# Anttwo/SuGaR

Hardware: AMD Instinct MI355X
Metric: train_step_images_per_sec (higher is better)
Workload: dtype f32; 1 GPU; metric: 1000000 Gaussians @ 1920x1080, SH degree 3, 3DGS train step (raster fwd -> 0.8 L1 + 0.2 DSSIM -> bwd -> Adam, 59 floats/Gaussian), 8 orbit cameras cycled; parallelism=view-sharded dp1, single process, no collective

## Files before the change

### include/sugar_raster.h

```cpp
#ifndef SUGAR_RASTER_H_INCLUDED
#define SUGAR_RASTER_H_INCLUDED

#include <stddef.h>
#include <stdint.h>

#ifdef __cplusplus
extern "C" {
#endif

#define SGR_ABI_VERSION 4

#define SGR_E_INVALID (-1)
#define SGR_E_HIP (-2)
#define SGR_E_ALLOC (-3)

typedef char* (*sgr_alloc_fn)(void* user, size_t bytes);

int sgr_abi_version(void);
const char* sgr_last_error(void);

int64_t sgr_forward(sgr_alloc_fn geom_alloc, void* geom_user,
                    sgr_alloc_fn binning_alloc, void* binning_user,
                    sgr_alloc_fn img_alloc, void* img_user,
                    int P, int D, int M,
// ... 13 lines not shown
#define SGR_HDR_L1_OVERFLOW 6
#define SGR_HDR_LAYOUT_CAP 8
#define SGR_HDR_DEEP 9
#define SGR_HDR_REPAIR 7
typedef struct sgr_forward_info {
    int binning_mode;
    int sync_free;
    int speculation;
} sgr_forward_info;
typedef struct sgr_forward_opts {
    int64_t binning_capacity;
    int flags;
    uint32_t* header_host;
    void* header_event;
    const uint32_t* tile_need;
    uint32_t* tile_need_out;
    float hint_margin;
    uint32_t chunk_grid;
    sgr_forward_info* info;
    const uint32_t* tile_order;
    uint32_t* tile_order_out;
} sgr_forward_opts;
int64_t sgr_forward_ex(sgr_alloc_fn geom_alloc, void* geom_user,
                       sgr_alloc_fn binning_alloc, void* binning_user,
                       sgr_alloc_fn img_alloc, void* img_user,
                       int P, int D, int M,
                       const float* background, int width, int height,
                       const float* means3D, const float* shs, const float* colors_precomp,
                       const float* opacities, const float* scales, float scale_modifier,
                       const float* rotations, const float* cov3D_precomp,
                       const float* viewmatrix, const float* projmatrix, const float* cam_pos,
                       float tan_fovx, float tan_fovy, int prefiltered,
                       float* out_color, int* radii, int debug, void* stream, const sgr_forward_opts* opts);

#define SGR_FLAG_RAW_PARAMS 1
#define SGR_FLAG_SINGLE_LEVEL_BINNING 2
#define SGR_FLAG_DEFER_POST 4
#define SGR_FLAG_SPECULATIVE 8
#define SGR_FLAG_EXACT_ALPHA 16
#define SGR_FLAG_NO_DEEP 32
#define SGR_FLAG_REACH 64
void sgr_set_deep_min(int entries);
int sgr_get_deep_min(void);
void sgr_set_exact_alpha(int on);
int sgr_get_exact_alpha(void);
#define SGR_MODE_RAW_PARAMS 4
#define SGR_MODE_SH_DIR_ELSEWHERE 8

int sgr_backward(int P, int D, int M, int64_t R,
                 const float* background, int width, int height,
                 const float* means3D, const float* shs, const float* colors_precomp,
                 const float* scales, float scale_modifier, const float* rotations,
                 const float* cov3D_precomp, const float* viewmatrix, const float* projmatrix,
                 const float* cam_pos, float tan_fovx, float tan_fovy, const int* radii,
                 char* geom_buffer, char* binning_buffer, char* img_buffer,
                 const float* dL_dpix,
                 float* dL_dmean2D, float* dL_dconic, float* dL_dopacity, float* dL_dcolor,
                 float* dL_dmean3D, float* dL_dcov3D, float* dL_dsh, float* dL_dscale, float* dL_drot,
                 int debug, void* stream);

int sgr_backward_phase(int phase, int P, int D, int M, int64_t R,
                       const float* background, int width, int height,
                       const float* means3D, const float* shs, const float* colors_precomp,
                       const float* scales, float scale_modifier, const float* rotations,
                       const float* cov3D_precomp, const float* viewmatrix, const float* projmatrix,
                       const float* cam_pos, float tan_fovx, float tan_fovy, const int* radii,
                       char* geom_buffer, char* binning_buffer, char* img_buffer,
                       const float* dL_dpix,
                       float* dL_dmean2D, float* dL_dconic, float* dL_dopacity, float* dL_dcolor,
                       float* dL_dmean3D, float* dL_dcov3D, float* dL_dsh, float* dL_dscale, float* dL_drot,
                       int debug, void* stream);

typedef struct sgr_backward_opts {
    float* max_radii2D;
    float* grad_accum;
    float* denom;
    float* campos_row;
    int flags;
} sgr_backward_opts;
#define SGR_BWD_EXACT_ALPHA 2
#define SGR_BWD_TILE_ORDER_READY 1
#define SGR_BWD_DENSE 8
#define SGR_BWD_ACC_CLEAN 4
int sgr_backward_ex(int phase, int P, int D, int M, int64_t R,
                    const float* background, int width, int height,
                    const float* means3D, const float* shs, const float* colors_precomp,
                    const float* scales, float scale_modifier, const float* rotations,
                    const float* cov3D_precomp, const float* viewmatrix, const float* projmatrix,
                    const float* cam_pos, float tan_fovx, float tan_fovy, const int* radii,
                    char* geom_buffer, char* binning_buffer, char* img_buffer,
                    const float* dL_dpix,
                    float* dL_dmean2D, float* dL_dconic, float* dL_dopacity, float* dL_dcolor,
                    float* dL_dmean3D, float* dL_dcov3D, float* dL_dsh, float* dL_dscale, float* dL_drot,
                    int debug, void* stream, const sgr_backward_opts* opts);

int sgr_sh_grad_from_views(int P, int n_views, int D, int M, const float* means3D, const float* campos_all,
                           const float* dcolor_all, int64_t view_stride, float* dL_dsh, void* stream);

int sgr_sh_adam_from_views(int P, int n_views, int D, int M, const float* means3D, const float* campos_all,
                           const float* dcolor_all, int64_t view_stride, float* sh_params, float* exp_avg, float* exp_avg_sq,
                           float lr_dc,
                           float lr_rest, float beta1, float beta2, float eps, int step, float grad_scale, void* stream);

int sgr_sh_adam_from_views_ex(int P, int n_views, int D, int M, const float* means3D, const float* campos_all,
                              const float* dcolor_all, int64_t view_stride, float* sh_params, float* exp_avg, float* exp_avg_sq,
                              float lr_dc, float lr_rest, float beta1, float beta2, float eps, int step, float grad_scale,
                              float* dmean_extra, void* stream);

int sgr_sh_adam_zero_grad(int P, int M, float* sh_params, float* exp_avg, float* exp_avg_sq, const uint8_t* reach, float lr_dc,
                          float lr_rest, float beta1, float beta2, float eps, int step, float grad_scale,
                          const uint32_t* guard_header, uint32_t guard_capacity, void* stream);
int sgr_sh_adam_from_views_masked(int P, int n_views, int D, int M, const float* means3D, const float* campos_all,
                                  const float* dcolor_all, int64_t view_stride, float* sh_params, float* exp_avg, float* exp_avg_sq,
                                  float lr_dc, float lr_rest, float beta1, float beta2, float eps, int step, float grad_scale,
                                  uint8_t* reach, const uint32_t* guard_header, uint32_t guard_capacity, void* stream);
void sgr_set_adam_overlap(int on);
int sgr_get_adam_overlap(void);
size_t sgr_geom_reach_offset_bytes(int P);

int sgr_mark_visible(int P, const float* means3D, const float* viewmatrix, const float* projmatrix,
                     uint8_t* present, void* stream);

size_t sgr_geom_bytes(int P);
size_t sgr_img_bytes(int width, int height);
size_t sgr_binning_bytes(int64_t R, int width, int height);

size_t sgr_geom_rec_offset(int P);
size_t sgr_geom_acc_offset_bytes(int P);
size_t sgr_img_final_T_offset(int width, int height);
size_t sgr_img_n_contrib_offset(int width, int height);
size_t sgr_img_tile_start_offset(int width, int height);
size_t sgr_img_tile_maxc_offset(int width, int height);
size_t sgr_img_tile_walked_offset(int width, int height);
size_t sgr_img_header_offset(int width, int height);
size_t sgr_binning_point_list_offset(int64_t R);

#define SGR_N_STAGES 15
void sgr_profile_enable(int stage_mask);
int sgr_profile_read(double* ms_sum, int64_t* count, int n_stages);


int sgr_dist2(int P, const float* points, float* meanDists, void* stream);
int sgr_knn(int N, const float* query, int M, const float* ref, int K, float* dists, int64_t* idx, void* stream);
size_t sgr_knn_grid_scratch_bytes(int M);
int sgr_knn_grid(int N, const float* query, int M, const float* ref, int K, float* dists, int64_t* idx, char* scratch,
                 void* stream);
int sgr_dist2_grid(int P, const float* points, float* meanDists, char* scratch, void* stream);

size_t sgr_l1_ssim_scratch_bytes(int channels, int width, int height);
int sgr_l1_ssim_forward(int channels, int width, int height, const float* img, const float* gt, float lambda,
                        char* scratch, float* loss_out, void* stream);
int sgr_l1_ssim_backward(int channels, int width, int height, const float* img, const float* gt, float lambda,
                         const char* scratch, const float* grad_loss, float* grad_img, void* stream);
int sgr_l1_ssim_backward_ex(int channels, int width, int height, const float* img, const float* gt, float lambda,
                            const char* scratch, const float* grad_loss, float* grad_img, float* loss_out, void* stream);

int sgr_adam_step(long long n, float* params, const float* grads, float* exp_avg, float* exp_avg_sq, int n_seg,
                  const long long* seg_begin, const long long* seg_end, const float* seg_lr_a, const float* seg_lr_b,
                  const int* seg_period, const int* seg_split, float beta1, float beta2, float eps, int step,
                  float grad_scale, void* stream);
int sgr_adam_step_multi(int n_tensors, const long long* n, float* const* params, const float* const* grads, float* const* exp_avg,
                        float* const* exp_avg_sq, const float* lr, const float* beta1, const float* beta2, const float* eps,
                        const int* step, void* stream);
int sgr_adam_step_ex(long long n, float* params, const float* grads, float* exp_avg, float* exp_avg_sq, int n_seg,
                     const long long* seg_begin, const long long* seg_end, const float* seg_lr_a, const float* seg_lr_b,
                     const int* seg_period, const int* seg_split, float beta1, float beta2, float eps, int step,
                     float grad_scale, const float* extra, long long extra_n, void* stream);

typedef struct sgr_train_config {
    int P, D, M, width, height;
    float* flat; float* flat_grad; float* exp_avg; float* exp_avg_sq;
    long long off_xyz, off_opacity, off_scaling, off_rotation, off_features, n_small;
    float lr_xyz, lr_opacity, lr_scaling, lr_rotation, lr_features_dc, lr_features_rest;
    float beta1, beta2, eps, lambda_dssim;
    const float* background;
    char* geom; size_t geom_bytes;
    char* img; size_t img_bytes;
    char* binning; size_t binning_bytes;
    int64_t binning_capacity;
    char* loss_scratch;
    float* image;
    float* grad_image;
    float* loss_out;
    float* colors;
    int* radii;
    uint32_t* header_host;
    float* dL_dmean2D;
    float* max_radii2D; float* grad_accum; float* denom;
} sgr_train_config;
typedef struct sgr_train_view {
    const float* viewmatrix; const float* projmatrix; const float* campos;
    float tan_fovx, tan_fovy;
    const float* gt_image;
    const uint32_t* tile_need;
    uint32_t* tile_need_out;
    float hint_margin;
    uint32_t chunk_grid;
    const uint32_t* tile_order;
    uint32_t* tile_order_out;
    uint32_t flags;
} sgr_train_view;
#define SGR_VIEW_DEEP_LISTS 1
typedef struct sgr_train_exchange {
    int n_views;
    const float* all_colors;
    int64_t view_stride;
    const float* all_campos;
    float grad_scale;
    int step;
    int64_t g_begin, g_end;
    int64_t f_begin, f_end;
} sgr_train_exchange;
typedef struct sgr_trainer sgr_trainer;
sgr_trainer* sgr_trainer_create(const sgr_train_config* cfg);
void sgr_trainer_destroy(sgr_trainer* t);
int sgr_trainer_set_binning(sgr_trainer* t, char* binning, size_t bytes, int64_t capacity);
int sgr_trainer_step(sgr_trainer* t, const sgr_train_view* view, int phases, const sgr_train_exchange* ex, void* stream);
int sgr_trainer_set_exchange_chunks(sgr_trainer* t, int n);
int sgr_trainer_forward_valid(sgr_trainer* t, uint32_t* header_out);
const char* sgr_trainer_last_error(void);
int sgr_trainer_acc_dirty(sgr_trainer* t);
int sgr_rccl_unique_id(char* out128);
int sgr_trainer_comm_init(sgr_trainer* t, const char* id128, int world, int rank, float* recv, size_t recv_bytes);
int sgr_trainer_comm_destroy(sgr_trainer* t);
int sgr_trainer_comm_abort(sgr_trainer* t);
int sgr_trainer_step_exchange(sgr_trainer* t, const sgr_train_view* view, int step, void* stream);
double sgr_trainer_last_exchange_wait_ms(sgr_trainer* t);
size_t sgr_bin2_bytes(int P, int width, int height);

int sgr_scaled_rotation_forward(int P, const float* quaternions, const float* scaling, int inverse_scales, float* out,
                                void* stream);
int sgr_scaled_rotation_backward(int P, const float* quaternions, const float* scaling, int inverse_scales,
                                 const float* dL_dout, float* dL_dquaternions, float* dL_dscaling, void* stream);

int sgr_pack_gaussians(int P, const float* centers, const float* inv_scaled_rot, const float* strengths, float* packed,
                       void* stream);
int sgr_density_field_forward(int N, int K, const float* x, const int64_t* nbr_idx, const float* centers,
                              const float* inv_scaled_rot, const float* strengths, float density_factor,
                              float* neighbor_opacities, float* density, const float* packed, void* stream);
int sgr_density_field_backward(int N, int K, const float* x, const int64_t* nbr_idx, const float* centers,
                               const float* inv_scaled_rot, const float* strengths, float density_factor,
                               const float* dL_dopacities, const float* dL_ddensity, float* dL_dx, float* dL_dcenters,
                               float* dL_dinv_scaled_rot, float* dL_dstrengths, const float* packed, void* stream);
size_t sgr_density_field_backward_scratch_bytes(int N, int K, int P);
int sgr_density_field_backward_gather(int N, int K, int P, const float* x, const int64_t* nbr_idx, const float* centers,
                                      const float* inv_scaled_rot, const float* strengths, float density_factor,
                                      const float* dL_dopacities, const float* dL_ddensity, float* dL_dx, float* dL_dcenters,
                                      float* dL_dinv_scaled_rot, float* dL_dstrengths, char* scratch, const float* packed, void* stream);

size_t sgr_scatter_add_rows_scratch_bytes(long long N, int P);
int sgr_scatter_add_rows(long long N, const int64_t* idx, const float* src, int W, int P, float* out, char* scratch, void* stream);

int sgr_sample_transform_forward(long long N, int P, const int64_t* idx, const float* points, const float* quaternions,
                                 const float* scaling, const float* noise, float factor, float* out, void* stream);
size_t sgr_sample_transform_backward_scratch_bytes(long long N, int P);
int sgr_sample_transform_backward(long long N, int P, const int64_t* idx, const float* quaternions, const float* scaling,
                                  const float* noise, float factor, const float* dL_dout, float* dL_dpoints, float* dL_dquaternions,
                                  float* dL_dscaling, char* scratch, void* stream);
int sgr_smallest_axis_forward(int P, const float* quaternions, const float* scaling, float* axis, int64_t* axis_idx, void* stream);
int sgr_smallest_axis_backward(int P, const float* quaternions, const float* scaling, const float* dL_daxis, float* dL_dquaternions,
                               void* stream);
int sgr_depth_lookup_forward(long long M, const float* points_cam, const float* projection, const float* depth, long long stride_y,
                             long long stride_x, int height, int width, float* out, void* stream);
int sgr_depth_lookup_backward(long long M, const float* points_cam, const float* projection, const float* depth, long long stride_y,
                              long long stride_x, int height, int width, const float* dL_dout, float* dL_dpoints_cam, float* dL_ddepth,
                              void* stream);
int sgr_sdf_field_forward(int N, int K, int P, const float* x, const int64_t* nbr_idx, const float* centers, const float* inv_scaled_rot,
                          const float* strengths, const float* min_scaling, float density_factor, float density_threshold,
                          float opacity_min_clamp, float* neighbor_opacities, float* density, float* beta, float* sdf,
                          const float* packed, void* stream);
size_t sgr_sdf_field_backward_scratch_bytes(int N, int K, int P);
int sgr_sdf_field_backward(int N, int K, int P, const float* x, const int64_t* nbr_idx, const float* centers, const float* inv_scaled_rot,
                           const float* strengths, float density_factor, float density_threshold, float opacity_min_clamp,
                           const float* density, const float* beta, const float* dL_dopacities, const float* dL_ddensity,
                           const float* dL_dbeta, const float* dL_dsdf, float* dL_dx, float* dL_dcenters, float* dL_dinv_scaled_rot,
                           float* dL_dstrengths, float* dL_dmin_scaling, char* scratch, const float* packed, void* stream);

#define SGR_CL_SQUARED_EST 1
#define SGR_CL_SQUARED_SURFACE 2
#define SGR_CL_WITH_EST 4
#define SGR_CL_WITH_SURFACE 8
int sgr_surface_band(int P, const float* points, const float* quaternions, const float* scaling, const float* world_to_view,
                     const float* cam_center, const float* projection, const float* depth, long long stride_y, long long stride_x,
                     int height, int width, float threshold, uint8_t* close, float* std_out, void* stream);
size_t sgr_estimation_loss_scratch_bytes(long long N);
int sgr_estimation_loss_forward(long long N, int P, int mode, int flags, const float* samples, const float* field, const float* beta,
                                const int64_t* sample_idx, const float* std, float scale, float clamp_max, const float* world_to_view,
                                const float* projection, const float* znear, const float* depth, long long stride_y, long long stride_x,
                                int height, int width, float* loss_estimation, float* loss_surface, int64_t* n_projected, char* scratch,
                                void* stream);
int sgr_estimation_loss_backward(long long N, int P, int mode, int flags, const float* samples, const float* field, const float* beta,
                                 const int64_t* sample_idx, const float* std, float scale, float clamp_max, const float* world_to_view,
                                 const float* projection, const float* znear, const float* depth, long long stride_y, long long stride_x,
                                 int height, int width, const int64_t* n_projected, const float* dL_dloss_estimation,
                                 const float* dL_dloss_surface, float* dL_dfield, float* dL_dbeta, float* dL_dsamples, float* dL_ddepth,
                                 void* stream);
size_t sgr_better_normal_forward_scratch_bytes(long long N, int K);
int sgr_better_normal_forward(long long N, int K, int P, const float* samples, const int64_t* sample_idx, const int64_t* knn_idx,
                              const float* normals, const float* points, const float* min_scaling, const float* opacities, float* loss,
                              char* scratch, void* stream);
size_t sgr_better_normal_backward_scratch_bytes(long long N, int K, int P, int through_normal_only);
int sgr_better_normal_backward(long long N, int K, int P, const float* samples, const int64_t* sample_idx, const int64_t* knn_idx,
                               const float* normals, const float* points, const float* min_scaling, const float* opacities,
                               int through_normal_only, const float* dL_dloss, float* dL_dnormals, float* dL_dpoints, float* dL_dsamples,
// ... 140 lines not shown
```

### sugar_amd/_lib.py

```python
from __future__ import annotations

import ctypes as C
import os

_HERE = os.path.dirname(os.path.abspath(__file__))
LIB_PATH = os.environ.get("SGR_LIB_PATH") or os.path.join(_HERE, "libsugar_raster.so")

ALLOC_FN = C.CFUNCTYPE(C.c_void_p, C.c_void_p, C.c_size_t)

_vp, _i, _f, _i64, _sz = C.c_void_p, C.c_int, C.c_float, C.c_int64, C.c_size_t
SIGNATURES = {
    "sgr_abi_version": (_i, []),
    "sgr_last_error": (C.c_char_p, []),
    "sgr_set_deep_min": (None, [_i]),
    "sgr_get_deep_min": (_i, []),
    "sgr_set_exact_alpha": (None, [_i]),
    "sgr_get_exact_alpha": (_i, []),
    "sgr_forward": (_i64, [ALLOC_FN, _vp, ALLOC_FN, _vp, ALLOC_FN, _vp, _i, _i, _i, _vp, _i, _i, _vp, _vp, _vp, _vp,
                           _vp, _f, _vp, _vp, _vp, _vp, _vp, _f, _f, _i, _vp, _vp, _i, _vp]),
    "sgr_forward_ex": (_i64, [ALLOC_FN, _vp, ALLOC_FN, _vp, ALLOC_FN, _vp, _i, _i, _i, _vp, _i, _i, _vp, _vp, _vp, _vp,
                              _vp, _f, _vp, _vp, _vp, _vp, _vp, _f, _f, _i, _vp, _vp, _i, _vp, _vp]),
    "sgr_backward": (_i, [_i, _i, _i, _i64, _vp, _i, _i, _vp, _vp, _vp, _vp, _f, _vp, _vp, _vp, _vp, _vp, _f, _f, _vp,
                          _vp, _vp, _vp, _vp, _vp, _vp, _vp, _vp, _vp, _vp, _vp, _vp, _vp, _i, _vp]),
    "sgr_backward_phase": (_i, [_i, _i, _i, _i, _i64, _vp, _i, _i, _vp, _vp, _vp, _vp, _f, _vp, _vp, _vp, _vp, _vp, _f, _f, _vp,
                                _vp, _vp, _vp, _vp, _vp, _vp, _vp, _vp, _vp, _vp, _vp, _vp, _vp, _i, _vp]),
    "sgr_backward_ex": (_i, [_i, _i, _i, _i, _i64, _vp, _i, _i, _vp, _vp, _vp, _vp, _f, _vp, _vp, _vp, _vp, _vp, _f, _f, _vp,
                             _vp, _vp, _vp, _vp, _vp, _vp, _vp, _vp, _vp, _vp, _vp, _vp, _vp, _i, _vp, _vp]),
    "sgr_mark_visible": (_i, [_i, _vp, _vp, _vp, _vp, _vp]),
    "sgr_trainer_create": (_vp, [_vp]),
    "sgr_trainer_destroy": (None, [_vp]),
    "sgr_trainer_set_binning": (_i, [_vp, _vp, _sz, _i64]),
    "sgr_trainer_step": (_i, [_vp, _vp, _i, _vp, _vp]),
    "sgr_trainer_forward_valid": (_i, [_vp, _vp]),
    "sgr_trainer_last_error": (C.c_char_p, []),
    "sgr_trainer_acc_dirty": (_i, [_vp]),
    "sgr_rccl_unique_id": (_i, [_vp]),
    "sgr_trainer_comm_init": (_i, [_vp, _vp, _i, _i, _vp, _sz]),
    "sgr_trainer_comm_destroy": (_i, [_vp]),
    "sgr_trainer_comm_abort": (_i, [_vp]),
    "sgr_trainer_step_exchange": (_i, [_vp, _vp, _i, _vp]),
    "sgr_trainer_set_exchange_chunks": (_i, [_vp, _i]),
    "sgr_trainer_last_exchange_wait_ms": (C.c_double, [_vp]),
    "sgr_bin2_bytes": (_sz, [_i, _i, _i]),
    "sgr_sh_grad_from_views": (_i, [_i, _i, _i, _i, _vp, _vp, _vp, _i64, _vp, _vp]),
    "sgr_sh_adam_from_views": (_i, [_i, _i, _i, _i, _vp, _vp, _vp, _i64, _vp, _vp, _vp, _f, _f, _f, _f, _f, _i, _f, _vp]),
    "sgr_sh_adam_from_views_ex": (_i, [_i, _i, _i, _i, _vp, _vp, _vp, _i64, _vp, _vp, _vp, _f, _f, _f, _f, _f, _i, _f, _vp, _vp]),
    "sgr_sh_adam_zero_grad": (_i, [_i, _i, _vp, _vp, _vp, _vp, _f, _f, _f, _f, _f, _i, _f, _vp, C.c_uint32, _vp]),
    "sgr_sh_adam_from_views_masked": (_i, [_i, _i, _i, _i, _vp, _vp, _vp, _i64, _vp, _vp, _vp, _f, _f, _f, _f, _f, _i, _f, _vp, _vp,
                                           C.c_uint32, _vp]),
    "sgr_set_adam_overlap": (None, [_i]),
    "sgr_get_adam_overlap": (_i, []),
    "sgr_geom_reach_offset_bytes": (_sz, [_i]),
    "sgr_geom_bytes": (_sz, [_i]),
    "sgr_img_bytes": (_sz, [_i, _i]),
    "sgr_binning_bytes": (_sz, [_i64, _i, _i]),
    "sgr_geom_rec_offset": (_sz, [_i]),
    "sgr_geom_acc_offset_bytes": (_sz, [_i]),
    "sgr_img_final_T_offset": (_sz, [_i, _i]),
    "sgr_img_n_contrib_offset": (_sz, [_i, _i]),
    "sgr_img_tile_start_offset": (_sz, [_i, _i]),
    "sgr_img_tile_maxc_offset": (_sz, [_i, _i]),
    "sgr_img_tile_walked_offset": (_sz, [_i, _i]),
    "sgr_img_header_offset": (_sz, [_i, _i]),
    "sgr_binning_point_list_offset": (_sz, [_i64]),
    "sgr_profile_enable": (None, [_i]),
    "sgr_profile_read": (_i, [_vp, _vp, _i]),
    "sgr_l1_ssim_scratch_bytes": (_sz, [_i, _i, _i]),
    "sgr_l1_ssim_forward": (_i, [_i, _i, _i, _vp, _vp, _f, _vp, _vp, _vp]),
    "sgr_l1_ssim_backward": (_i, [_i, _i, _i, _vp, _vp, _f, _vp, _vp, _vp, _vp]),
    "sgr_l1_ssim_backward_ex": (_i, [_i, _i, _i, _vp, _vp, _f, _vp, _vp, _vp, _vp, _vp]),
    "sgr_adam_step": (_i, [C.c_longlong, _vp, _vp, _vp, _vp, _i, _vp, _vp, _vp, _vp, _vp, _vp, _f, _f, _f, _i, _f, _vp]),
    "sgr_adam_step_multi": (_i, [_i, _vp, _vp, _vp, _vp, _vp, _vp, _vp, _vp, _vp, _vp, _vp]),
    "sgr_adam_step_ex": (_i, [C.c_longlong, _vp, _vp, _vp, _vp, _i, _vp, _vp, _vp, _vp, _vp, _vp, _f, _f, _f, _i, _f, _vp, C.c_longlong, _vp]),
    "sgr_density_field_forward": (_i, [_i, _i, _vp, _vp, _vp, _vp, _vp, _f, _vp, _vp, _vp, _vp]),
    "sgr_density_field_backward": (_i, [_i, _i, _vp, _vp, _vp, _vp, _vp, _f, _vp, _vp, _vp, _vp, _vp, _vp, _vp, _vp]),
    "sgr_density_field_backward_scratch_bytes": (_sz, [_i, _i, _i]),
    "sgr_scatter_add_rows_scratch_bytes": (_sz, [C.c_longlong, _i]),
    "sgr_scatter_add_rows": (_i, [C.c_longlong, _vp, _vp, _i, _i, _vp, _vp, _vp]),
    "sgr_density_field_backward_gather": (_i, [_i, _i, _i, _vp, _vp, _vp, _vp, _vp, _f, _vp, _vp, _vp, _vp, _vp, _vp, _vp, _vp, _vp]),
    "sgr_sample_transform_forward": (_i, [C.c_longlong, _i, _vp, _vp, _vp, _vp, _vp, _f, _vp, _vp]),
    "sgr_sample_transform_backward_scratch_bytes": (_sz, [C.c_longlong, _i]),
    "sgr_sample_transform_backward": (_i, [C.c_longlong, _i, _vp, _vp, _vp, _vp, _f, _vp, _vp, _vp, _vp, _vp, _vp]),
    "sgr_smallest_axis_forward": (_i, [_i, _vp, _vp, _vp, _vp, _vp]),
    "sgr_smallest_axis_backward": (_i, [_i, _vp, _vp, _vp, _vp, _vp]),
    "sgr_depth_lookup_forward": (_i, [C.c_longlong, _vp, _vp, _vp, C.c_longlong, C.c_longlong, _i, _i, _vp, _vp]),
    "sgr_depth_lookup_backward": (_i, [C.c_longlong, _vp, _vp, _vp, C.c_longlong, C.c_longlong, _i, _i, _vp, _vp, _vp, _vp]),
    "sgr_sdf_field_forward": (_i, [_i, _i, _i, _vp, _vp, _vp, _vp, _vp, _vp, _f, _f, _f, _vp, _vp, _vp, _vp, _vp, _vp]),
    "sgr_sdf_field_backward_scratch_bytes": (_sz, [_i, _i, _i]),
    "sgr_sdf_field_backward": (_i, [_i, _i, _i, _vp, _vp, _vp, _vp, _vp, _f, _f, _f, _vp, _vp, _vp, _vp, _vp, _vp, _vp, _vp, _vp, _vp,
                                    _vp, _vp, _vp, _vp]),
    "sgr_surface_band": (_i, [_i] + [_vp] * 7 + [C.c_longlong, C.c_longlong, _i, _i, _f, _vp, _vp, _vp]),
    "sgr_estimation_loss_scratch_bytes": (_sz, [C.c_longlong]),
    "sgr_estimation_loss_forward": (_i, [C.c_longlong, _i, _i, _i] + [_vp] * 5 + [_f, _f] + [_vp] * 4 + [C.c_longlong, C.c_longlong, _i, _i]
                                    + [_vp] * 5),
    "sgr_estimation_loss_backward": (_i, [C.c_longlong, _i, _i, _i] + [_vp] * 5 + [_f, _f] + [_vp] * 4 + [C.c_longlong, C.c_longlong, _i, _i]
                                     + [_vp] * 8),
    "sgr_better_normal_forward_scratch_bytes": (_sz, [C.c_longlong, _i]),
    "sgr_better_normal_forward": (_i, [C.c_longlong, _i, _i] + [_vp] * 10),
    "sgr_better_normal_backward_scratch_bytes": (_sz, [C.c_longlong, _i, _i, _i]),
    "sgr_better_normal_backward": (_i, [C.c_longlong, _i, _i] + [_vp] * 7 + [_i] + [_vp] * 6),
    "sgr_opacity_entropy_scratch_bytes": (_sz, [_i]),
    "sgr_opacity_entropy_forward": (_i, [_i] + [_vp] * 6),
    "sgr_opacity_entropy_backward": (_i, [_i] + [_vp] * 6),
    "sgr_draw_samples_scratch_bytes": (_sz, [_i]),
    "sgr_draw_samples": (_i, [_i, _vp, C.c_longlong, C.c_uint64, C.c_uint64, _vp, _vp, _vp, _vp, _vp]),
    "sgr_scaled_rotation_forward": (_i, [_i, _vp, _vp, _i, _vp, _vp]),
    "sgr_scaled_rotation_backward": (_i, [_i, _vp, _vp, _i, _vp, _vp, _vp, _vp]),
    "sgr_pack_gaussians": (_i, [_i, _vp, _vp, _vp, _vp, _vp]),
    "sgr_view_std": (_i, [_i, _vp, _vp, _vp, _vp, _vp, _vp]),
    "sgr_view_depth_rgb": (_i, [_i, _vp, _vp, _vp, _vp]),
    "sgr_unproject_pixels": (_i, [_i, _vp, _vp, _i, _i, _f, _f, _vp, _vp, _vp]),
    "sgr_pick_pixels_scratch_bytes": (_sz, [_i]),
    "sgr_pick_pixels": (_i, [_i, _vp, _i, C.c_uint32, _vp, _vp, _vp, _vp, _vp]),
    "sgr_compact_level_rows": (_i, [_i, _i, _vp, _vp, _vp, _vp, _vp, _vp, _vp, _vp, _vp, _vp, _vp, _vp, _vp, _vp]),
    "sgr_compact_level_rows_scratch_bytes": (_sz, [_i, _i]),
    "sgr_level_set_points": (_i, [_i, _i, _vp, _vp, _vp, _vp, _vp, _vp, _vp, _i, _vp, _i, _f, _f, _vp, _vp, _vp, _vp, _vp]),
    "sgr_sh_to_rgb_forward": (_i, [_i, _i, _i, _vp, _vp, _vp, _i, _vp, _vp, _vp]),
    "sgr_sh_to_rgb_backward": (_i, [_i, _i, _i, _vp, _vp, _vp, _i, _vp, _vp, _vp, _vp, _vp, _vp]),
    "sgr_activations_forward": (_i, [_i, _vp, _vp, _vp, _vp, _vp, _vp, _vp]),
    "sgr_activations_backward": (_i, [_i, _vp, _vp, _vp, _vp, _vp, _vp, _vp, _vp, _vp, _vp]),
    "sgr_dist2": (_i, [_i, _vp, _vp, _vp]),
    "sgr_knn": (_i, [_i, _vp, _i, _vp, _i, _vp, _vp, _vp]),
    "sgr_knn_grid_scratch_bytes": (_sz, [_i]),
    "sgr_knn_grid": (_i, [_i, _vp, _i, _vp, _i, _vp, _vp, _vp, _vp]),
    "sgr_dist2_grid": (_i, [_i, _vp, _vp, _vp, _vp]),
    "sgr_rasterize_meshes_scratch_bytes": (_sz, [_i64, _i, _i]),
    "sgr_splat_mesh_face_verts": (_i, [_i, _vp, _vp, _vp, _vp, _f, _vp, _vp, _vp, _vp]),
    "sgr_texture_size": (_i, [_i, _i]),
    "sgr_texture_atlas": (_i, [_i, _i, _i, _i, _vp, _vp, _vp, _vp, _vp, _i, _i, _vp, _vp, _vp, _vp]),
    "sgr_texture_bake_view": (_i, [_i, _i, _i, _vp, _vp, _vp, _vp, _f, _f, _i, _vp, _vp, _i64, _i64, _i64, _i, _vp, _vp, _vp, _vp]),
    "sgr_texture_finalize": (_i, [_i, _vp, _vp, _vp, _vp]),
    "sgr_shade_texture_uv": (_i, [_i, _i, _i, _i64, _vp, _vp, _vp, _vp, _i64, _vp, _i64, _vp, _vp, _i, _i, _i, _i, _vp, _vp, _f, _f, _f, _f,
                                  _vp, _vp]),
    "sgr_mesh_bind_forward": (_i, [_i, _i, _i, _vp, _vp, _vp, _vp, _vp, _vp, _vp, _vp, _vp, _vp]),
    "sgr_mesh_bind_backward": (_i, [_i, _i, _i, _vp, _vp, _vp, _vp, _vp, _vp, _vp, _vp, _vp, _vp, _vp, _vp, _vp, _vp, _vp]),
    "sgr_normal_consistency_scratch_bytes": (_sz, []),
    "sgr_normal_consistency_forward": (_i, [_i, _i, _vp, _vp, _vp, _vp, _vp]),
    "sgr_normal_consistency_backward": (_i, [_i, _i, _vp, _vp, _vp, _vp, _vp, _vp, _vp, _vp]),
    "sgr_marching_cubes_scratch_bytes": (_sz, [_i, _i, _i]),
    "sgr_marching_cubes_count": (_i, [_i, _i, _i, _vp, _f, _vp, _vp, _vp]),
    "sgr_marching_cubes_emit": (_i, [_i, _i, _i, _vp, _f, _vp, _i64, _i64, _vp, _vp, _vp]),
    "sgr_mesh_vertex_normals": (_i, [_i, _i64, _vp, _vp, _vp, _vp, _vp, _vp]),
    "sgr_grid_points": (_i, [_i, _i, _i, _vp, _vp, _vp, _i64, _i64, _vp, _vp]),
    "sgr_mesh_decimate_quadrics": (_i, [_i, _i, _vp, _vp, _vp, _vp, _vp, C.c_double, _vp, _vp]),
    "sgr_mesh_decimate_edges": (_i, [_i, _i, _vp, _vp, _vp, _vp, _vp, _vp, _vp, _vp, _vp, _vp, _vp]),
    "sgr_mesh_decimate_eval": (_i, [_i, _i, _vp, _vp, _vp, _vp, _vp, _vp, _vp, _vp, _vp, _vp, _vp, _vp, _vp, _vp, _vp]),
    "sgr_mesh_decimate_select": (_i, [_i, _i, _vp, _vp, _vp, _vp, _vp, _vp, _vp, _vp, _vp, _vp, _vp, _vp, _vp]),
    "sgr_mesh_decimate_apply": (_i, [_i, _i, _vp, _vp, _vp, _vp, _vp, _vp, _vp, _vp, _vp, _vp, _vp, _vp]),
    "sgr_mesh_decimate_compact": (_i, [_i, _i, _vp, _vp, _vp, _vp, _vp, _vp, _vp, _vp, _vp, _vp, _vp, _vp, _vp]),
    "sgr_mesh_clean_degenerate": (_i, [_i, _vp, _vp, _vp]),
    "sgr_mesh_clean_duplicate_faces": (_i, [_i, _vp, _vp, _vp, _vp]),
    "sgr_mesh_clean_duplicate_verts": (_i, [_i, _vp, _vp, _vp, _vp]),
    "sgr_mesh_clean_nonmanifold": (_i, [_i, _i, _vp, _vp, _vp, _vp, _vp, _vp]),
    "sgr_mesh_clean_referenced": (_i, [_i, _i, _vp, _vp, _vp]),
    "sgr_sparse_sweep_mark": (_i, [_i, _vp, _i, _f, _i, _i, _i, _vp, _vp, _vp, _vp, _vp, _vp, _vp, _vp]),
    "sgr_sparse_sweep_compact": (_i, [_i, _i, _i, _vp, _vp, _vp, _i, _f, _f, _vp, _vp, _vp, _vp]),
    "sgr_sparse_sweep_points": (_i, [_i, _i, _i, _vp, _vp, _vp, _vp, _i, _i, _vp, _vp]),
    "sgr_sparse_sweep_scatter": (_i, [_i, _i, _i, _vp, _i, _i, _vp, _vp, _vp]),
    "sgr_point_surface_mark": (_i, [_i, _vp, _f, _i, _i, _i, _vp, _vp, _vp, _vp, _vp, _vp]),
    "sgr_point_surface_pack": (_i, [_i, _vp, _vp, _vp, _vp]),
    "sgr_point_surface_eval": (_i, [C.c_longlong, _i, _vp, _vp, _i, _vp, _f, _vp, _vp, _vp]),
    "sgr_point_surface_spurious": (_i, [_i, _vp, _i, _i, _i, _vp, _vp, _vp]),
    "sgr_mesh_peel_border_scratch_bytes": (_sz, [_i]),
    "sgr_mesh_peel_border": (_i, [_i, _i, _vp, _vp, _vp, _i, _vp, _vp, _vp]),
    "sgr_rasterize_meshes": (_i64, [_vp, _i64, _i64, _i, _i, _f, _i, _i, _i, _i, _vp, _sz, ALLOC_FN, _vp, _vp, _vp, _vp, _vp, _vp]),
}

ABI_VERSION = 4


class ForwardInfo(C.Structure):
    _fields_ = [("binning_mode", _i), ("sync_free", _i), ("speculation", _i)]


class ForwardOpts(C.Structure):
    _fields_ = [("binning_capacity", _i64), ("flags", _i), ("header_host", _vp), ("header_event", _vp), ("tile_need", _vp),
                ("tile_need_out", _vp), ("hint_margin", _f), ("chunk_grid", C.c_uint32), ("info", C.POINTER(ForwardInfo)),
                ("tile_order", _vp), ("tile_order_out", _vp)]


class BackwardOpts(C.Structure):
    _fields_ = [("max_radii2D", _vp), ("grad_accum", _vp), ("denom", _vp), ("campos_row", _vp), ("flags", _i)]


class TrainConfig(C.Structure):
    _fields_ = [("P", _i), ("D", _i), ("M", _i), ("width", _i), ("height", _i),
                ("flat", _vp), ("flat_grad", _vp), ("exp_avg", _vp), ("exp_avg_sq", _vp),
                ("off_xyz", C.c_longlong), ("off_opacity", C.c_longlong), ("off_scaling", C.c_longlong),
                ("off_rotation", C.c_longlong), ("off_features", C.c_longlong), ("n_small", C.c_longlong),
                ("lr_xyz", _f), ("lr_opacity", _f), ("lr_scaling", _f), ("lr_rotation", _f), ("lr_features_dc", _f),
                ("lr_features_rest", _f), ("beta1", _f), ("beta2", _f), ("eps", _f), ("lambda_dssim", _f),
                ("background", _vp), ("geom", _vp), ("geom_bytes", _sz), ("img", _vp), ("img_bytes", _sz), ("binning", _vp),
                ("binning_bytes", _sz), ("binning_capacity", _i64), ("loss_scratch", _vp), ("image", _vp), ("grad_image", _vp),
                ("loss_out", _vp), ("colors", _vp), ("radii", _vp), ("header_host", _vp), ("dL_dmean2D", _vp),
                ("max_radii2D", _vp), ("grad_accum", _vp), ("denom", _vp)]


class TrainView(C.Structure):
    _fields_ = [("viewmatrix", _vp), ("projmatrix", _vp), ("campos", _vp), ("tan_fovx", _f), ("tan_fovy", _f), ("gt_image", _vp),
                ("tile_need", _vp), ("tile_need_out", _vp), ("hint_margin", _f), ("chunk_grid", C.c_uint32),
                ("tile_order", _vp), ("tile_order_out", _vp), ("flags", C.c_uint32)]


class TrainExchange(C.Structure):
    _fields_ = [("n_views", _i), ("all_colors", _vp), ("view_stride", _i64), ("all_campos", _vp), ("grad_scale", _f), ("step", _i),
                ("g_begin", _i64), ("g_end", _i64), ("f_begin", _i64), ("f_end", _i64)]


SGR_FLAG_RAW_PARAMS, SGR_FLAG_SINGLE_LEVEL_BINNING, SGR_FLAG_SPECULATIVE = 1, 2, 8
SGR_BWD_TILE_ORDER_READY, SGR_BWD_ACC_CLEAN, SGR_BWD_DENSE = 1, 4, 8
HDR_R, HDR_HINT_MISS, HDR_L1_OVERFLOW = 0, 3, 6

_lib = None


def load() -> C.CDLL:
    global _lib
    if _lib is not None:
        return _lib
    if not os.path.exists(LIB_PATH):
        raise ImportError(
            f"{LIB_PATH} not found: the gfx950 HIP rasterizer is not built. Run `python -m sugar_amd.build` "
            "(or __graft_entry__.build()). There is no CPU fallback.")
    lib = C.CDLL(LIB_PATH)
    for name, (res, args) in SIGNATURES.items():
        try:
            fn = getattr(lib, name)
        except AttributeError as e:
            raise ImportError(f"{LIB_PATH} does not export `{name}` (ABI mismatch; rebuild)") from e
        fn.restype = res
        fn.argtypes = args
    if lib.sgr_abi_version() != ABI_VERSION:
        raise ImportError(f"sugar_raster ABI version mismatch: library {lib.sgr_abi_version()}, bindings {ABI_VERSION} (rebuild)")
    _lib = lib
    return lib


def last_error() -> str:
    return load().sgr_last_error().decode(errors="replace")
```

### sugar_amd/csrc/capi.hip

```cpp
#include "../../include/sugar_raster.h"
#include "sgr_common.h"
#include "tile_order.h"

#include <cstdlib>
#include <mutex>
#include <string>
#include <vector>

namespace {

thread_local std::string g_err;

int fail(int code, const std::string& msg)
{
    g_err = msg;
    return code;
}

#define HIP_TRY(expr)                                                                                   \
    do {                                                                                                \
        hipError_t e_ = (expr);                                                                         \
        if (e_ != hipSuccess)                                                                           \
            return fail(SGR_E_HIP, std::string(#expr) + ": " + hipGetErrorString(e_));                  \
    } while (0)
// ... 22 lines not shown
SideStream* side_stream()
{
    int dev = 0;
    if (hipGetDevice(&dev) != hipSuccess || dev < 0 || dev >= 16) return nullptr;
    SideStream& sd = g_side[dev];
    if (!sd.st) {
        int lo = 0, hi = 0;
        (void)hipDeviceGetStreamPriorityRange(&lo, &hi);
        if (hipStreamCreateWithPriority(&sd.st, hipStreamNonBlocking, hi) != hipSuccess) { sd.st = nullptr; (void)hipGetLastError(); return nullptr; }
        if (hipEventCreateWithFlags(&sd.fork, hipEventDisableTiming) != hipSuccess ||
            hipEventCreateWithFlags(&sd.join, hipEventDisableTiming) != hipSuccess) { (void)hipGetLastError(); return nullptr; }
        sd.device = dev;
    }
    return (sd.fork && sd.join) ? &sd : nullptr;
}

struct Prof {
    unsigned mask = 0;
    struct Rec { int stage; hipEvent_t a, b; };
    std::vector<Rec> recs;
    std::vector<hipEvent_t> pool;
    hipEvent_t get()
    {
        if (!pool.empty()) { hipEvent_t e = pool.back(); pool.pop_back(); return e; }
        hipEvent_t e = nullptr;
        (void)hipEventCreate(&e);
        return e;
    }
};
Prof g_prof;
std::mutex g_prof_mu;

}

SgrStageTimer::SgrStageTimer(hipStream_t s_, int stage_) : s(s_), stage(stage_)
{
    if (g_prof.mask & (1u << stage_)) {
        std::lock_guard<std::mutex> lk(g_prof_mu);
        if (g_prof.recs.size() < 65536) {
            a = g_prof.get(); b = g_prof.get();
            live = a && b;
        }
        if (live) (void)hipEventRecord(a, s);
    }
}
void SgrStageTimer::stop()
{
    if (live) {
        (void)hipEventRecord(b, s);
        std::lock_guard<std::mutex> lk(g_prof_mu);
        g_prof.recs.push_back({stage, a, b});
        live = false;
    }
}

int sgr_fail(int code, const char* msg) { return fail(code, msg ? msg : ""); }

static int g_exact_alpha = -1;
int sgr_exact_alpha()
{
    if (g_exact_alpha < 0) { const char* e = getenv("SGR_EXACT_ALPHA"); g_exact_alpha = (e && e[0] == '0') ? 0 : 1; }
    return g_exact_alpha;
}

static int g_deep_min = -1;
uint32_t sgr_deep_min()
{
    if (g_deep_min < 0) { const char* e = getenv("SGR_DEEP_MIN"); g_deep_min = e ? atoi(e) : 0; if (g_deep_min < 0) g_deep_min = 0; }
    return (uint32_t)g_deep_min;
}

static int g_adam_overlap = -1;
int sgr_adam_overlap()
{
    if (g_adam_overlap < 0) { const char* e = getenv("SGR_ADAM_OVERLAP"); g_adam_overlap = e ? (e[0] == '2' ? 2 : (e[0] != '0' ? 1 : 0)) : SGR_ADAM_OVERLAP_DEFAULT; }
    return g_adam_overlap;
}
int sgr_adam_overlap_k()
{
    static int k = -1;
    if (k < 0) { const char* e = getenv("SGR_ADAM_OVERLAP_K"); k = e ? atoi(e) : 24; if (k < 8 || (k & 7)) k = 24; }
    return k;
}

extern "C" {

int sgr_abi_version(void) { return SGR_ABI_VERSION; }
void sgr_set_adam_overlap(int on) { g_adam_overlap = on == 2 ? 2 : (on ? 1 : 0); }
int sgr_get_adam_overlap(void) { return sgr_adam_overlap(); }
size_t sgr_geom_reach_offset_bytes(int P) { return sgr_geom_reach_offset(P); }
void sgr_set_deep_min(int entries) { g_deep_min = entries > 0 ? entries : 0; }
int sgr_get_deep_min(void) { return (int)sgr_deep_min(); }
void sgr_set_exact_alpha(int on) { g_exact_alpha = on ? 1 : 0; }
int sgr_get_exact_alpha(void) { return sgr_exact_alpha(); }

const char* sgr_last_error(void) { return g_err.c_str(); }

size_t sgr_geom_bytes(int P) { return sgr_geom_total(P); }
size_t sgr_img_bytes(int width, int height) { return sgr_img_layout(width, height).total; }
size_t sgr_binning_bytes(int64_t R, int width, int height) { return sgr_bin_layout(R, sgr_img_layout(width, height).T).total; }
size_t sgr_geom_rec_offset(int) { return 0; }
size_t sgr_geom_acc_offset_bytes(int P) { return sgr_geom_acc_offset(P); }
size_t sgr_img_final_T_offset(int w, int h) { return sgr_img_layout(w, h).final_T; }
size_t sgr_img_n_contrib_offset(int w, int h) { return sgr_img_layout(w, h).n_contrib; }
size_t sgr_img_tile_start_offset(int w, int h) { return sgr_img_layout(w, h).tile_start; }
size_t sgr_img_tile_maxc_offset(int w, int h) { return sgr_img_layout(w, h).tile_maxc; }
size_t sgr_img_tile_walked_offset(int w, int h) { return sgr_img_layout(w, h).tile_walked; }
size_t sgr_img_header_offset(int w, int h) { return sgr_img_layout(w, h).header; }
size_t sgr_binning_point_list_offset(int64_t R) { return sgr_bin_layout(R, 0).point_list; }

void sgr_profile_enable(int stage_mask) { g_prof.mask = (unsigned)stage_mask; }

int sgr_profile_read(double* ms_sum, int64_t* count, int n_stages)
{
    std::lock_guard<std::mutex> lk(g_prof_mu);
    for (int i = 0; i < n_stages; i++) { ms_sum[i] = 0.0; count[i] = 0; }
    for (auto& r : g_prof.recs) {
        float ms = 0.f;
        hipError_t e = hipEventSynchronize(r.b);
        if (e == hipSuccess) e = hipEventElapsedTime(&ms, r.a, r.b);
        if (e == hipSuccess && r.stage < n_stages) { ms_sum[r.stage] += ms; count[r.stage]++; }
        g_prof.pool.push_back(r.a); g_prof.pool.push_back(r.b);
    }
    g_prof.recs.clear();
    return 0;
}

int sgr_mark_visible(int P, const float* means3D, const float* viewmatrix, const float* projmatrix, uint8_t* present,
                     void* stream)
{
    (void)projmatrix;
    hipStream_t s = (hipStream_t)stream;
    if (P < 0) return fail(SGR_E_INVALID, "P < 0");
    sgr_launch_mark_visible(P, means3D, viewmatrix, present, s);
    hipError_t e = hipGetLastError();
    if (e != hipSuccess) return fail(SGR_E_HIP, std::string("mark_visible: ") + hipGetErrorString(e));
    return 0;
}

int64_t sgr_forward_ex(sgr_alloc_fn geom_alloc, void* geom_user, sgr_alloc_fn binning_alloc, void* binning_user,
                       sgr_alloc_fn img_alloc, void* img_user, int P, int D, int M, const float* background, int width,
                       int height, const float* means3D, const float* shs, const float* colors_precomp,
                       const float* opacities, const float* scales, float scale_modifier, const float* rotations,
                       const float* cov3D_precomp, const float* viewmatrix, const float* projmatrix, const float* cam_pos,
                       float tan_fovx, float tan_fovy, int prefiltered, float* out_color, int* radii, int debug,
                       void* stream, const sgr_forward_opts* opts)
{
    (void)prefiltered;
    hipStream_t s = (hipStream_t)stream;
    static const sgr_forward_opts no_opts = {0, 0, nullptr, nullptr, nullptr, nullptr, 0.f, 0u, nullptr};
    if (!opts) opts = &no_opts;
    int64_t binning_capacity = opts->binning_capacity;
    const int flags = opts->flags;
    const int binning_mode = (flags & SGR_FLAG_SINGLE_LEVEL_BINNING) ? 1 : 0;
    const int exact = (sgr_exact_alpha() || (flags & SGR_FLAG_EXACT_ALPHA)) ? 1 : 0;
    if (opts->tile_need && binning_mode == 1) return fail(SGR_E_INVALID, "the walk hint needs the two-level binning");
    if (P <= 0 || width <= 0 || height <= 0) return fail(SGR_E_INVALID, "P, width and height must be positive");
    if (!means3D || !opacities || !viewmatrix || !projmatrix || !background || !out_color)
        return fail(SGR_E_INVALID, "null required pointer");
    if (!shs && !colors_precomp) return fail(SGR_E_INVALID, "need SHs or precomputed colours");
    if (shs && !colors_precomp && (M <= 0 || M > 16 || (D + 1) * (D + 1) > M || D < 0 || D > 3))
        return fail(SGR_E_INVALID, "SH degree / coefficient count out of range (D <= 3, (D+1)^2 <= M <= 16)");
    if (shs && !colors_precomp && !cam_pos) return fail(SGR_E_INVALID, "cam_pos required with SHs");
    if (!cov3D_precomp && (!scales || !rotations)) return fail(SGR_E_INVALID, "need scales+rotations or cov3D_precomp");

    const ImgLayout IL = sgr_img_layout(width, height);
    const bool legacy_ok = IL.n_blocks > 0;
    if (IL.gx > 65535 || IL.gy > 65535) return fail(SGR_E_INVALID, "image too large: more than 65535 tiles per axis");
    if (!legacy_ok && binning_mode == 1)
        return fail(SGR_E_INVALID, "image too large for the single-level binning (one LDS counter per tile, about 38 000 tiles)");
// ... 206 lines not shown
        if (opts->tile_need && !two_level) return fail(SGR_E_INVALID, "the walk hint needs the two-level binning (level-1 overflow on this view)");
        rc = tail(R, false, n_chunks);
        if (rc < 0) return rc;
    }
    return R;
}

int64_t sgr_forward(sgr_alloc_fn geom_alloc, void* geom_user, sgr_alloc_fn binning_alloc, void* binning_user,
                    sgr_alloc_fn img_alloc, void* img_user, int P, int D, int M, const float* background, int width,
                    int height, const float* means3D, const float* shs, const float* colors_precomp,
                    const float* opacities, const float* scales, float scale_modifier, const float* rotations,
                    const float* cov3D_precomp, const float* viewmatrix, const float* projmatrix, const float* cam_pos,
                    float tan_fovx, float tan_fovy, int prefiltered, float* out_color, int* radii, int debug,
                    void* stream)
{
    return sgr_forward_ex(geom_alloc, geom_user, binning_alloc, binning_user, img_alloc, img_user, P, D, M, background, width, height,
                          means3D, shs, colors_precomp, opacities, scales, scale_modifier, rotations, cov3D_precomp, viewmatrix,
                          projmatrix, cam_pos, tan_fovx, tan_fovy, prefiltered, out_color, radii, debug, stream, nullptr);
}

int sgr_forward_post_job(int width, int height, char* img_buffer, int64_t R, const sgr_forward_opts* opts, SgrTileOrderJob* job)
{
    if (!img_buffer || !opts || !job) return SGR_E_INVALID;
    const ImgLayout IL = sgr_img_layout(width, height);
    uint32_t* hh_dev = nullptr;
    if (opts->header_host && hipHostGetDevicePointer(reinterpret_cast<void**>(&hh_dev), opts->header_host, 0) != hipSuccess) return SGR_E_INVALID;
    job->T = IL.T;
    job->list_cap = (uint32_t)(R > 0xFFFFFFFFll ? 0xFFFFFFFFll : R);
    job->tile_maxc = reinterpret_cast<const uint32_t*>(img_buffer + IL.tile_maxc);
    job->tile_walked = opts->tile_need_out ? reinterpret_cast<const uint32_t*>(img_buffer + IL.tile_walked) : nullptr;
    job->header = reinterpret_cast<const uint32_t*>(img_buffer + IL.header);
    job->order = reinterpret_cast<uint32_t*>(img_buffer + IL.tile_cursor);
    job->order_copy = opts->tile_order_out;
    job->need_out = opts->tile_need_out;
    job->header_host = hh_dev;
    job->margin = opts->hint_margin > 0.f ? opts->hint_margin : 0.25f;
    job->gx = IL.gx;
    job->gy = IL.gy;
    return 0;
}

}
hipError_t sgr_acc_reset(char* geom_buffer, int P, hipStream_t s)
{
    SgrStageTimer t(s, SGR_STAGE_FILL);
    return hipMemsetAsync(geom_buffer + sgr_geom_acc_offset(P), 0, (size_t)P * SGR_ACC_STRIDE * 4, s);
}
extern "C" {

static int backward_impl(int phase, int P, int D, int M, int64_t R, const float* background, int width, int height,
                         const float* means3D, const float* shs, const float* colors_precomp, const float* scales,
                         float scale_modifier, const float* rotations, const float* cov3D_precomp, const float* viewmatrix,
                         const float* projmatrix, const float* cam_pos, float tan_fovx, float tan_fovy, char* geom_buffer,
                         char* binning_buffer, char* img_buffer, const float* dL_dpix, float* dL_dmean2D, float* dL_dconic,
                         float* dL_dopacity, float* dL_dcolor, float* dL_dmean3D, float* dL_dcov3D, float* dL_dsh,
                         float* dL_dscale, float* dL_drot, int debug, void* stream, const sgr_backward_opts* opts = nullptr,
                         const SgrShAdamJob* job = nullptr)
{
    hipStream_t s = (hipStream_t)stream;
    const int raw_params = (phase & SGR_MODE_RAW_PARAMS) ? 1 : 0;
    const int sh_dir_elsewhere = (phase & SGR_MODE_SH_DIR_ELSEWHERE) ? 1 : 0;
    phase &= 3;
    if (phase < 0 || phase > 2) return fail(SGR_E_INVALID, "phase must be 0, 1 or 2");
    if (P <= 0 || width <= 0 || height <= 0) return fail(SGR_E_INVALID, "P, width and height must be positive");
    if (!geom_buffer || !binning_buffer || !img_buffer || !dL_dpix) return fail(SGR_E_INVALID, "null scratch / dL_dpix");
    if (!dL_dopacity || !dL_dcolor || !dL_dmean3D) return fail(SGR_E_INVALID, "null gradient output");
    if (cov3D_precomp && !dL_dcov3D) return fail(SGR_E_INVALID, "dL_dcov3D required with cov3D_precomp");
    const bool use_sh = shs && !colors_precomp;
    const bool compact = use_sh && !dL_dsh;
    if (!cov3D_precomp && (!dL_dscale || !dL_drot)) return fail(SGR_E_INVALID, "dL_dscale/dL_drot required");
    if (phase == 1 && !compact) return fail(SGR_E_INVALID, "the two-phase backward is for the compact SH mode");

    const ImgLayout IL = sgr_img_layout(width, height);
    const BinLayout BL = sgr_bin_layout(R, IL.T);
    const GeomRec* rec = reinterpret_cast<const GeomRec*>(geom_buffer);
    const float* final_T = reinterpret_cast<const float*>(img_buffer + IL.final_T);
    const uint32_t* n_contrib = reinterpret_cast<const uint32_t*>(img_buffer + IL.n_contrib);
    const uint32_t* tile_start = reinterpret_cast<const uint32_t*>(img_buffer + IL.tile_start);
    const uint32_t* blk_nb = reinterpret_cast<const uint32_t*>(img_buffer + IL.blk_nb);
    const uint32_t* point_list = reinterpret_cast<const uint32_t*>(binning_buffer + BL.point_list);

    float* acc = reinterpret_cast<float*>(geom_buffer + sgr_geom_acc_offset(P));
    const bool acc_clean = opts && (opts->flags & SGR_BWD_ACC_CLEAN);
    if (phase != 2) {
        if (!acc_clean) HIP_TRY(sgr_acc_reset(geom_buffer, P, s));
        if (R > 0) {
            SgrStageTimer t(s, SGR_STAGE_BLEND_BWD);
            sgr_launch_blend_bwd(width, height, IL.gx, IL.gy, tile_start, point_list, binning_buffer, blk_nb, rec, background, final_T,
                                 n_contrib, dL_dpix, acc, reinterpret_cast<const uint32_t*>(img_buffer + IL.tile_maxc),
                                 reinterpret_cast<const uint32_t*>(img_buffer + IL.header), (uint32_t)(R > 0xFFFFFFFFll ? 0xFFFFFFFFll : R),
                                 reinterpret_cast<uint32_t*>(img_buffer + IL.tile_cursor),
                                 (opts && (opts->flags & SGR_BWD_TILE_ORDER_READY)) ? 1 : 0, s,
                                 (sgr_exact_alpha() || (opts && (opts->flags & SGR_BWD_EXACT_ALPHA))) ? 1 : 0, job);
        } else if (job) {
            sgr_launch_sh_adam_zero(*job, s);
        }
        STAGE_CHECK("blend_bwd");
        if (phase == 1) {
            { SgrStageTimer t(s, SGR_STAGE_MASKED_COLORS); sgr_launch_masked_colors(P, rec, acc, dL_dcolor, cam_pos, opts ? opts->campos_row : nullptr, s); }
            STAGE_CHECK("masked_colors");
            return 0;
        }
    }
    PreprocessBwdArgs pb;
    pb.P = P; pb.D = D; pb.M = use_sh ? M : 0;
    pb.means3D = means3D; pb.shs = use_sh ? shs : nullptr;
    pb.scales = cov3D_precomp ? nullptr : scales; pb.rotations = cov3D_precomp ? nullptr : rotations;
    pb.scale_modifier = scale_modifier; pb.cov3D_precomp = cov3D_precomp;
    pb.viewmatrix = viewmatrix; pb.projmatrix = projmatrix; pb.cam_pos = cam_pos;
    pb.W = width; pb.H = height; pb.tan_fovx = tan_fovx; pb.tan_fovy = tan_fovy;
    pb.focal_y = height / (2.0f * tan_fovy);
    pb.focal_x = width / (2.0f * tan_fovx);
    pb.rec = rec;
    pb.raw_params = raw_params && !cov3D_precomp;
    pb.sh_dir_elsewhere = sh_dir_elsewhere && use_sh && !dL_dsh;
    pb.acc = acc;
    pb.acc_clean = acc_clean ? 1 : 0;
    pb.dense = (opts && (opts->flags & SGR_BWD_DENSE)) ? 1 : 0;
    pb.header = reinterpret_cast<const uint32_t*>(img_buffer + IL.header);
    pb.list_cap = (uint32_t)(R > 0xFFFFFFFFll ? 0xFFFFFFFFll : R);
    pb.campos_row = (opts && compact && phase == 0) ? opts->campos_row : nullptr;
    pb.dens_max_radii = opts ? opts->max_radii2D : nullptr;
    pb.dens_accum = opts ? opts->grad_accum : nullptr;
    pb.dens_denom = opts ? opts->denom : nullptr;
    pb.dL_dmean2D = dL_dmean2D; pb.dL_dconic = dL_dconic; pb.dL_dopacity = dL_dopacity;
    pb.dL_dcolor = phase == 2 ? nullptr : dL_dcolor;
    pb.dL_dmean3D = dL_dmean3D; pb.dL_dcov3D = dL_dcov3D; pb.dL_dsh = use_sh ? dL_dsh : nullptr;
    pb.dL_dscale = cov3D_precomp ? nullptr : dL_dscale; pb.dL_drot = cov3D_precomp ? nullptr : dL_drot;
    { SgrStageTimer t(s, SGR_STAGE_PREPROCESS_BWD); sgr_launch_preprocess_bwd(pb, s); }
    STAGE_CHECK("preprocess_bwd");
    return 0;
}

int sgr_backward(int P, int D, int M, int64_t R, const float* background, int width, int height, const float* means3D,
                 const float* shs, const float* colors_precomp, const float* scales, float scale_modifier,
                 const float* rotations, const float* cov3D_precomp, const float* viewmatrix, const float* projmatrix,
                 const float* cam_pos, float tan_fovx, float tan_fovy, const int* radii, char* geom_buffer,
                 char* binning_buffer, char* img_buffer, const float* dL_dpix, float* dL_dmean2D, float* dL_dconic,
                 float* dL_dopacity, float* dL_dcolor, float* dL_dmean3D, float* dL_dcov3D, float* dL_dsh,
                 float* dL_dscale, float* dL_drot, int debug, void* stream)
{
    (void)radii;
    return backward_impl(0, P, D, M, R, background, width, height, means3D, shs, colors_precomp, scales, scale_modifier, rotations,
                         cov3D_precomp, viewmatrix, projmatrix, cam_pos, tan_fovx, tan_fovy, geom_buffer, binning_buffer, img_buffer,
                         dL_dpix, dL_dmean2D, dL_dconic, dL_dopacity, dL_dcolor, dL_dmean3D, dL_dcov3D, dL_dsh, dL_dscale, dL_drot,
                         debug, stream);
}

int sgr_backward_phase(int phase, int P, int D, int M, int64_t R, const float* background, int width, int height,
                       const float* means3D, const float* shs, const float* colors_precomp, const float* scales,
                       float scale_modifier, const float* rotations, const float* cov3D_precomp, const float* viewmatrix,
                       const float* projmatrix, const float* cam_pos, float tan_fovx, float tan_fovy, const int* radii,
                       char* geom_buffer, char* binning_buffer, char* img_buffer, const float* dL_dpix, float* dL_dmean2D,
                       float* dL_dconic, float* dL_dopacity, float* dL_dcolor, float* dL_dmean3D, float* dL_dcov3D, float* dL_dsh,
                       float* dL_dscale, float* dL_drot, int debug, void* stream)
{
    (void)radii;
    return backward_impl(phase, P, D, M, R, background, width, height, means3D, shs, colors_precomp, scales, scale_modifier,
                         rotations, cov3D_precomp, viewmatrix, projmatrix, cam_pos, tan_fovx, tan_fovy, geom_buffer, binning_buffer,
                         img_buffer, dL_dpix, dL_dmean2D, dL_dconic, dL_dopacity, dL_dcolor, dL_dmean3D, dL_dcov3D, dL_dsh, dL_dscale,
                         dL_drot, debug, stream);
}

int sgr_backward_ex(int phase, int P, int D, int M, int64_t R, const float* background, int width, int height,
                    const float* means3D, const float* shs, const float* colors_precomp, const float* scales,
                    float scale_modifier, const float* rotations, const float* cov3D_precomp, const float* viewmatrix,
                    const float* projmatrix, const float* cam_pos, float tan_fovx, float tan_fovy, const int* radii,
                    char* geom_buffer, char* binning_buffer, char* img_buffer, const float* dL_dpix, float* dL_dmean2D,
                    float* dL_dconic, float* dL_dopacity, float* dL_dcolor, float* dL_dmean3D, float* dL_dcov3D, float* dL_dsh,
                    float* dL_dscale, float* dL_drot, int debug, void* stream, const sgr_backward_opts* opts)
{
    (void)radii;
    return backward_impl(phase, P, D, M, R, background, width, height, means3D, shs, colors_precomp, scales, scale_modifier,
                         rotations, cov3D_precomp, viewmatrix, projmatrix, cam_pos, tan_fovx, tan_fovy, geom_buffer, binning_buffer,
                         img_buffer, dL_dpix, dL_dmean2D, dL_dconic, dL_dopacity, dL_dcolor, dL_dmean3D, dL_dcov3D, dL_dsh, dL_dscale,
                         dL_drot, debug, stream, opts);
}

void sgr_debug_bin2_offsets(int P, int width, int height, size_t* out)
{
    const ImgLayout IL = sgr_img_layout(width, height);
    const Bin2Layout B = sgr_bin2_layout(P, IL.gx, IL.gy);
    out[0] = IL.total + B.sup_start; out[1] = IL.total + B.chunk_base; out[2] = IL.total + B.cnt2; out[3] = IL.total + B.chunk_sup;
    out[4] = (size_t)B.T1; out[5] = (size_t)B.sgx; out[6] = (size_t)B.chunk_cap; out[7] = IL.header;
}

size_t sgr_bin2_bytes(int P, int width, int height)
{
    const ImgLayout IL = sgr_img_layout(width, height);
    return sgr_bin2_layout(P, IL.gx, IL.gy).total;
}

int sgr_sh_grad_from_views(int P, int n_views, int D, int M, const float* means3D, const float* campos_all,
                           const float* dcolor_all, int64_t view_stride, float* dL_dsh, void* stream)
{
    if (P <= 0) return 0;
    if (n_views <= 0 || D < 0 || D > 3 || M < (D + 1) * (D + 1) || M > 16 || !means3D || !campos_all || !dcolor_all || !dL_dsh)
        return fail(SGR_E_INVALID, "sgr_sh_grad_from_views: bad arguments");
    if (view_stride != 0 && view_stride < P) return fail(SGR_E_INVALID, "sgr_sh_grad_from_views: view_stride < P");
    sgr_launch_sh_grad_from_views(P, n_views, D, M, (size_t)(view_stride ? view_stride : P), means3D, campos_all, dcolor_all, dL_dsh,
                                  (hipStream_t)stream);
// ... 93 lines not shown
```

### sugar_amd/csrc/preprocess.hip

```cpp
#include "../../include/sugar_raster.h"
#include "sgr_common.h"
#include "sh_adam_update.h"

namespace {

__device__ __constant__ const float SH_C0 = 0.28209479177387814f;
__device__ __constant__ const float SH_C1 = 0.4886025119029199f;
__device__ __constant__ const float SH_C2[5] = {1.0925484305920792f, -1.0925484305920792f, 0.31539156525252005f,
                                                 -1.0925484305920792f, 0.5462742152960396f};
__device__ __constant__ const float SH_C3[7] = {-0.5900435899266435f, 2.890611442640554f, -0.4570457994644658f,
                                                 0.3731763325901154f, -0.4570457994644658f, 1.445305721320277f,
                                                 -0.5900435899266435f};

__device__ __forceinline__ float fmin_(float a, float b) { return a < b ? a : b; }
__device__ __forceinline__ float fmax_(float a, float b) { return a > b ? a : b; }

__device__ __forceinline__ int f2i_sat(float v)
{
    if (v != v) return 0;
    if (v >= 2147483648.0f) return 2147483647;
    if (v <= -2147483648.0f) return (-2147483647 - 1);
    return (int)v;
}

// ... 335 lines not shown
                    rec.r = fmax_(c0, 0.0f); rec.g = fmax_(c1, 0.0f); rec.b = fmax_(c2, 0.0f);
                }
                rec.x = pix_x; rec.y = pix_y; rec.cx = conx; rec.cy = cony; rec.cz = conz;
                rec.opacity = a.raw_params ? sigmoid_(op_in) : op_in;
                rec.depth = p_view.z;
                rec.radius = r_int;
                out_radius = r_int;
            }
        }
    }
    const uint32_t key = out_radius > 0 ? __float_as_uint(rec.depth) : 0xFFFFFFFFu;
    if (valid) {
        float4* dst = reinterpret_cast<float4*>(a.rec + idx);
        const float4* srcv = reinterpret_cast<const float4*>(&rec);
        dst[0] = srcv[0]; dst[1] = srcv[1]; dst[2] = srcv[2];
        if (a.radii) a.radii[idx] = out_radius;
        if (!a.keys_elsewhere) a.sort_keys[idx] = key;
        a.rect_by_id[idx] = rect;
    }
    if (a.keys_elsewhere) return;
    uint32_t kmin = key, kmax = key == 0xFFFFFFFFu ? 0u : key;
    for (int o = 32; o > 0; o >>= 1) {
        kmin = min(kmin, (uint32_t)__shfl_xor((int)kmin, o));
        kmax = max(kmax, (uint32_t)__shfl_xor((int)kmax, o));
    }
    if ((threadIdx.x & 63) == 0) { s_mm[0][threadIdx.x >> 6] = kmin; s_mm[1][threadIdx.x >> 6] = kmax; }
    __syncthreads();
    if (threadIdx.x == 0)
        a.key_minmax[blockIdx.x] = make_uint2(min(min(s_mm[0][0], s_mm[0][1]), min(s_mm[0][2], s_mm[0][3])),
                                              max(max(s_mm[1][0], s_mm[1][1]), max(s_mm[1][2], s_mm[1][3])));
}

__global__ void __launch_bounds__(256) k_depth_keys(PreprocessArgs a)
{
    __shared__ uint32_t s_mm[2][4];
    const int idx = blockIdx.x * 256 + threadIdx.x;
    const bool valid = idx < a.P;
    const size_t i3 = 3 * (size_t)(valid ? idx : a.P - 1);
    if (blockIdx.x == 0)
        for (int i = threadIdx.x; i < a.n_sort_counters; i += 256) a.sort_counters[i] = 0u;
    const float cam_raw = cam_request(a.viewmatrix, a.projmatrix, a.cam_pos);
    const V3 p_orig = {a.means3D[i3], a.means3D[i3 + 1], a.means3D[i3 + 2]};
    Cam cam;
    cam_unpack(cam_raw, cam);
    const V3 p_view = xform4x3(p_orig, cam.vm);
    const uint32_t key = (valid && !(p_view.z <= 0.2f)) ? __float_as_uint(p_view.z) : 0xFFFFFFFFu;
    if (valid) a.sort_keys[idx] = key;
    uint32_t kmin = key, kmax = key == 0xFFFFFFFFu ? 0u : key;
    for (int o = 32; o > 0; o >>= 1) {
        kmin = min(kmin, (uint32_t)__shfl_xor((int)kmin, o));
        kmax = max(kmax, (uint32_t)__shfl_xor((int)kmax, o));
    }
    if ((threadIdx.x & 63) == 0) { s_mm[0][threadIdx.x >> 6] = kmin; s_mm[1][threadIdx.x >> 6] = kmax; }
    __syncthreads();
    if (threadIdx.x == 0)
        a.key_minmax[blockIdx.x] = make_uint2(min(min(s_mm[0][0], s_mm[0][1]), min(s_mm[0][2], s_mm[0][3])),
                                              max(max(s_mm[1][0], s_mm[1][1]), max(s_mm[1][2], s_mm[1][3])));
}

#ifndef SGR_PRE_BWD_BLOCKS
#define SGR_PRE_BWD_BLOCKS 3
#endif
struct BwdHead { float4 rec0, rec1, rec2, s0, s1; float s2x; };
__device__ __forceinline__ void bwd_head_load(const PreprocessBwdArgs& a, int idx, BwdHead& h)
{
    const float4* rp4 = reinterpret_cast<const float4*>(a.rec + idx);
    h.rec0 = rp4[0]; h.rec1 = rp4[1]; h.rec2 = rp4[2];
    const float4* ap = reinterpret_cast<const float4*>(a.acc + SGR_ACC_STRIDE * (size_t)idx);
    h.s0 = ap[0]; h.s1 = ap[1];
    h.s2x = a.acc[SGR_ACC_STRIDE * (size_t)idx + 8];
}
__device__ __forceinline__ bool bwd_touched(const float4 s0, const float4 s1, const float s2x)
{
    return !(s0.x == 0.f && s0.y == 0.f && s0.z == 0.f && s0.w == 0.f && s1.x == 0.f && s1.y == 0.f && s1.z == 0.f && s1.w == 0.f &&
             s2x == 0.f);
}
__device__ __forceinline__ void bwd_acc_clean(const PreprocessBwdArgs& a, int idx)
{
    float4* ap = reinterpret_cast<float4*>(a.acc + SGR_ACC_STRIDE * (size_t)idx);
    const float4 z4 = {0.f, 0.f, 0.f, 0.f};
    ap[0] = z4; ap[1] = z4;
    a.acc[SGR_ACC_STRIDE * (size_t)idx + 8] = 0.f;
}
template <bool STORE_SH>
__device__ __forceinline__ void bwd_zero_row(const PreprocessBwdArgs& a, int idx, float* __restrict__ stage, bool stats, int radius)
{
    const size_t i3 = 3 * (size_t)idx;
    const int n_sh = a.M * 3;
    if (a.dL_dmean2D) { a.dL_dmean2D[i3] = 0; a.dL_dmean2D[i3 + 1] = 0; a.dL_dmean2D[i3 + 2] = 0; }
    if (a.dL_dconic) { float4 z4 = {0, 0, 0, 0}; *reinterpret_cast<float4*>(a.dL_dconic + 4 * (size_t)idx) = z4; }
    a.dL_dopacity[idx] = 0;
    if (a.dL_dcolor) { a.dL_dcolor[i3] = 0; a.dL_dcolor[i3 + 1] = 0; a.dL_dcolor[i3 + 2] = 0; }
    a.dL_dmean3D[i3] = 0; a.dL_dmean3D[i3 + 1] = 0; a.dL_dmean3D[i3 + 2] = 0;
    if (a.dL_dcov3D) for (int k = 0; k < 6; k++) a.dL_dcov3D[6 * (size_t)idx + k] = 0;
    if (STORE_SH) {
        if (stage) {
#pragma unroll
            for (int k = 0; k < 48; k++) stage[65 * k] = 0.0f;
        } else {
            for (int k = 0; k < n_sh; k++) a.dL_dsh[(size_t)idx * n_sh + k] = 0;
        }
    }
    if (a.dL_dscale) { a.dL_dscale[i3] = 0; a.dL_dscale[i3 + 1] = 0; a.dL_dscale[i3 + 2] = 0; }
    if (a.dL_drot) { float4 z = {0, 0, 0, 0}; *reinterpret_cast<float4*>(a.dL_drot + 4 * (size_t)idx) = z; }
    if (stats) {
        if (a.dens_denom) a.dens_denom[idx] += 1.0f;
        if (a.dens_max_radii) a.dens_max_radii[idx] = fmaxf(a.dens_max_radii[idx], (float)radius);
    }
}

template <bool STORE_SH, int SH>
__device__ __forceinline__ void bwd_full_row(const PreprocessBwdArgs& a, const int idx, const BwdHead& h, const Cam& cam,
                                             float* __restrict__ stage)
{
    const size_t i3 = 3 * (size_t)idx;
    const float4 rec0 = h.rec0, rec1 = h.rec1, rec2 = h.rec2, s0 = h.s0, s1 = h.s1;
    const float s2x = h.s2x;
    const V3 mean = {a.means3D[i3], a.means3D[i3 + 1], a.means3D[i3 + 2]};
    float sc[3] = {0, 0, 0}, q[4] = {0, 0, 0, 0};
    float4 q_raw = make_float4(0.f, 0.f, 0.f, 0.f);
    float c6[6];
    if (a.cov3D_precomp) {
#pragma unroll
        for (int k = 0; k < 6; k++) c6[k] = a.cov3D_precomp[6 * (size_t)idx + k];
    } else {
        sc[0] = a.scales[i3]; sc[1] = a.scales[i3 + 1]; sc[2] = a.scales[i3 + 2];
        q_raw = *reinterpret_cast<const float4*>(a.rotations + 4 * (size_t)idx);
    }
    const int radius = __float_as_int(rec1.w);
    const uint32_t clamped = __float_as_uint(rec2.w);
    const float* v = cam.vm;
    float dmean[3] = {0, 0, 0}, dcov[6] = {0, 0, 0, 0, 0, 0};
    const int n_sh = a.M * 3;
    float sh[48];
    if (SH != 2) load_sh<48, SH == 0>(a.shs, idx, a.M, sh);
    if (!a.cov3D_precomp) {
        float4 q4 = q_raw;
        if (a.raw_params) {
            sc[0] = expf(sc[0]); sc[1] = expf(sc[1]); sc[2] = expf(sc[2]);
            const float inv = 1.0f / fmaxf(quat_norm_contracted(q4), 1e-12f);
            q4 = make_float4(q4.x * inv, q4.y * inv, q4.z * inv, q4.w * inv);
        }
        q[0] = q4.x; q[1] = q4.y; q[2] = q4.z; q[3] = q4.w;
        cov3d_from_scale_rot(sc, a.scale_modifier, q, c6);
    }
    float dcol[3], dm2x, dm2y;
    float g0, g1, g3;
    {
        const float op = rec1.y, cx = rec0.z, cy = rec0.w, cz = rec1.x;
        dcol[0] = s0.x; dcol[1] = s0.y; dcol[2] = s0.z;
        const float ddelx_dx = 0.5f * a.W, ddely_dy = 0.5f * a.H;
        dm2x = -(op * ddelx_dx) * (cx * s1.x + cy * s1.y);
        dm2y = -(op * ddely_dy) * (cz * s1.y + cy * s1.x);
        g0 = -0.5f * op * s1.z; g1 = -0.5f * op * s1.w; g3 = -0.5f * op * s2x;
        if (a.dL_dmean2D) { a.dL_dmean2D[i3] = dm2x; a.dL_dmean2D[i3 + 1] = dm2y; a.dL_dmean2D[i3 + 2] = 0; }
        if (a.dens_accum) a.dens_accum[idx] += sqrtf(dm2x * dm2x + dm2y * dm2y);
        if (a.dens_denom) a.dens_denom[idx] += 1.0f;
        if (a.dens_max_radii) a.dens_max_radii[idx] = fmaxf(a.dens_max_radii[idx], (float)radius);
        float4 gc = {g0, g1, 0.f, g3};
        if (a.dL_dconic) *reinterpret_cast<float4*>(a.dL_dconic + 4 * (size_t)idx) = gc;
        a.dL_dopacity[idx] = a.raw_params ? s0.w * op * (1.0f - op) : s0.w;
        if (a.dL_dcolor) {
            const bool mk = a.sh_dir_elsewhere != 0;
            a.dL_dcolor[i3] = (mk && (clamped & 1u)) ? 0.f : dcol[0];
            a.dL_dcolor[i3 + 1] = (mk && (clamped & 2u)) ? 0.f : dcol[1];
            a.dL_dcolor[i3 + 2] = (mk && (clamped & 4u)) ? 0.f : dcol[2];
        }
    }
    {
        float T[2][3], txtz, tytz; V3 t;
        compute_T(mean, a.focal_x, a.focal_y, a.tan_fovx, a.tan_fovy, v, T, t, txtz, tytz);
        const float limx = 1.3f * a.tan_fovx, limy = 1.3f * a.tan_fovy;
        const float x_grad_mul = (txtz < -limx || txtz > limx) ? 0.0f : 1.0f;
        const float y_grad_mul = (tytz < -limy || tytz > limy) ? 0.0f : 1.0f;
        float ca, cb, cc;
        cov2d_from_T(T, c6, ca, cb, cc);
        ca += 0.3f; cc += 0.3f;
        float denom = ca * cc - cb * cb;
        float dL_da = 0, dL_db = 0, dL_dc = 0;
        float denom2inv = 1.0f / ((denom * denom) + 0.0000001f);
        float V[3][3] = {{c6[0], c6[1], c6[2]}, {c6[1], c6[3], c6[4]}, {c6[2], c6[4], c6[5]}};
        if (denom2inv != 0) {
            dL_da = denom2inv * (-cc * cc * g0 + 2 * cb * cc * g1 + (denom - ca * cc) * g3);
            dL_dc = denom2inv * (-ca * ca * g3 + 2 * ca * cb * g1 + (denom - ca * cc) * g0);
            dL_db = denom2inv * 2 * (cb * cc * g0 - (denom + 2 * cb * cb) * g1 + ca * cb * g3);
            dcov[0] = (T[0][0] * T[0][0] * dL_da + T[0][0] * T[1][0] * dL_db + T[1][0] * T[1][0] * dL_dc);
            dcov[3] = (T[0][1] * T[0][1] * dL_da + T[0][1] * T[1][1] * dL_db + T[1][1] * T[1][1] * dL_dc);
            dcov[5] = (T[0][2] * T[0][2] * dL_da + T[0][2] * T[1][2] * dL_db + T[1][2] * T[1][2] * dL_dc);
            dcov[1] = 2 * T[0][0] * T[0][1] * dL_da + (T[0][0] * T[1][1] + T[0][1] * T[1][0]) * dL_db + 2 * T[1][0] * T[1][1] * dL_dc;
            dcov[2] = 2 * T[0][0] * T[0][2] * dL_da + (T[0][0] * T[1][2] + T[0][2] * T[1][0]) * dL_db + 2 * T[1][0] * T[1][2] * dL_dc;
// ... 68 lines not shown
        for (int c = 0; c < 3; c++) {
            float h[16];
#pragma unroll
            for (int k = 0; k < 16; k++) h[k] = sh[3 * k + c];
            float dRGBdx, dRGBdy, dRGBdz;
            sh_dir_channel(deg, h, x, y, z, dRGBdx, dRGBdy, dRGBdz);
            dL_ddir[0] += dRGBdx * dLm[c]; dL_ddir[1] += dRGBdy * dLm[c]; dL_ddir[2] += dRGBdz * dLm[c];
        }
        {
            V3 vv = dir_orig;
            float sum2 = vv.x * vv.x + vv.y * vv.y + vv.z * vv.z;
            float invsum32 = 1.0f / sqrtf(sum2 * sum2 * sum2);
            float ox = ((+sum2 - vv.x * vv.x) * dL_ddir[0] - vv.y * vv.x * dL_ddir[1] - vv.z * vv.x * dL_ddir[2]) * invsum32;
            float oy = (-vv.x * vv.y * dL_ddir[0] + (sum2 - vv.y * vv.y) * dL_ddir[1] - vv.z * vv.y * dL_ddir[2]) * invsum32;
            float oz = (-vv.x * vv.z * dL_ddir[0] - vv.y * vv.z * dL_ddir[1] + (sum2 - vv.z * vv.z) * dL_ddir[2]) * invsum32;
            dmean[0] += ox; dmean[1] += oy; dmean[2] += oz;
        }
        if (!STORE_SH && a.dL_dcolor) {
            a.dL_dcolor[i3] = ((clamped >> 0) & 1u) ? 0.f : dcol[0];
            a.dL_dcolor[i3 + 1] = ((clamped >> 1) & 1u) ? 0.f : dcol[1];
            a.dL_dcolor[i3 + 2] = ((clamped >> 2) & 1u) ? 0.f : dcol[2];
        }
    }
    if (a.scales) {
        float r = q[0], x = q[1], y = q[2], z = q[3];
        float R[3][3], M[3][3];
        quat_to_glmR(q, R);
        float s[3] = {a.scale_modifier * sc[0], a.scale_modifier * sc[1], a.scale_modifier * sc[2]};
#pragma unroll
        for (int c = 0; c < 3; c++)
#pragma unroll
            for (int k = 0; k < 3; k++) M[c][k] = s[k] * R[c][k];
        const float* d = dcov;
        float Dm[3][3] = {{d[0], 0.5f * d[1], 0.5f * d[2]}, {0.5f * d[1], d[3], 0.5f * d[4]}, {0.5f * d[2], 0.5f * d[4], d[5]}};
        float X[3][3], dM[3][3], dMt[3][3];
#pragma unroll
        for (int c = 0; c < 3; c++)
#pragma unroll
            for (int k = 0; k < 3; k++) X[c][k] = 2.0f * M[c][k];
#pragma unroll
        for (int c = 0; c < 3; c++)
#pragma unroll
            for (int rr = 0; rr < 3; rr++) dM[c][rr] = X[0][rr] * Dm[c][0] + X[1][rr] * Dm[c][1] + X[2][rr] * Dm[c][2];
#pragma unroll
        for (int c = 0; c < 3; c++)
#pragma unroll
            for (int rr = 0; rr < 3; rr++) dMt[c][rr] = dM[rr][c];
#pragma unroll
        for (int k = 0; k < 3; k++) {
            const float ds = R[0][k] * dMt[k][0] + R[1][k] * dMt[k][1] + R[2][k] * dMt[k][2];
            a.dL_dscale[i3 + k] = a.raw_params ? ds * sc[k] : ds;
        }
#pragma unroll
        for (int k = 0; k < 3; k++)
#pragma unroll
            for (int rr = 0; rr < 3; rr++) dMt[k][rr] *= s[k];
        float4 dq;
        dq.x = 2 * z * (dMt[0][1] - dMt[1][0]) + 2 * y * (dMt[2][0] - dMt[0][2]) + 2 * x * (dMt[1][2] - dMt[2][1]);
        dq.y = 2 * y * (dMt[1][0] + dMt[0][1]) + 2 * z * (dMt[2][0] + dMt[0][2]) + 2 * r * (dMt[1][2] - dMt[2][1]) - 4 * x * (dMt[2][2] + dMt[1][1]);
        dq.z = 2 * x * (dMt[1][0] + dMt[0][1]) + 2 * r * (dMt[2][0] - dMt[0][2]) + 2 * z * (dMt[1][2] + dMt[2][1]) - 4 * y * (dMt[2][2] + dMt[0][0]);
        dq.w = 2 * r * (dMt[0][1] - dMt[1][0]) + 2 * x * (dMt[2][0] + dMt[0][2]) + 2 * y * (dMt[1][2] + dMt[2][1]) - 4 * z * (dMt[1][1] + dMt[0][0]);
        if (a.raw_params) {
            const float n = quat_norm_contracted(q_raw);
            if (n > 1e-12f) {
                const float inv = 1.0f / n;
                const float nx = q_raw.x * inv, ny = q_raw.y * inv, nz = q_raw.z * inv, nw = q_raw.w * inv;
                const float dot = __builtin_fmaf(nw, dq.w, __builtin_fmaf(nz, dq.z, __builtin_fmaf(ny, dq.y, nx * dq.x)));
                dq = make_float4(__builtin_fmaf(-nx, dot, dq.x) * inv, __builtin_fmaf(-ny, dot, dq.y) * inv,
                                 __builtin_fmaf(-nz, dot, dq.z) * inv, __builtin_fmaf(-nw, dot, dq.w) * inv);
            } else {
                dq = make_float4(dq.x * 1e12f, dq.y * 1e12f, dq.z * 1e12f, dq.w * 1e12f);
            }
        }
        *reinterpret_cast<float4*>(a.dL_drot + 4 * (size_t)idx) = dq;
    }
    a.dL_dmean3D[i3] = dmean[0]; a.dL_dmean3D[i3 + 1] = dmean[1]; a.dL_dmean3D[i3 + 2] = dmean[2];
    if (a.dL_dcov3D) {
#pragma unroll
        for (int k = 0; k < 6; k++) a.dL_dcov3D[6 * (size_t)idx + k] = dcov[k];
    }
}

template <bool STORE_SH, int SH>
__device__ __forceinline__ void preprocess_bwd_lane(const PreprocessBwdArgs& a, float* __restrict__ stage, const int idx0)
{
    if (a.campos_row && idx0 < 3) a.campos_row[idx0] = a.cam_pos[idx0];
    uint32_t hdr_r = 0u, hdr_miss = 0u, hdr_ovf = 0u;
    if (a.header) { hdr_r = a.header[SGR_HDR_R]; hdr_miss = a.header[SGR_HDR_HINT_MISS]; hdr_ovf = a.header[4 + SGR_B2_HDR_OVERFLOW]; }
    const bool valid = idx0 < a.P;
    const int idx = valid ? idx0 : a.P - 1;
    const float cam_raw = cam_request(a.viewmatrix, a.projmatrix, a.cam_pos);
    BwdHead h;
    bwd_head_load(a, idx, h);
    Cam cam;
    cam_unpack(cam_raw, cam);
    if (a.acc_clean) {
        const bool dirty = valid && bwd_touched(h.s0, h.s1, h.s2x);
        const unsigned long long m = __ballot(dirty);
        if (__popcll(m) >= 32) {
            const int lane = threadIdx.x & 63;
            const long long row0 = (long long)idx0 - lane;
            float4* w4 = reinterpret_cast<float4*>(a.acc + SGR_ACC_STRIDE * (size_t)row0);
            const float4 z4 = {0.f, 0.f, 0.f, 0.f};
#pragma unroll
            for (int i = 0; i < 4; i++) {
                const int j = i * 64 + lane;
                if (row0 + (j >> 2) < (long long)a.P) w4[j] = z4;
            }
        } else if (dirty) {
            bwd_acc_clean(a, idx);
        }
    }
    if (!valid) return;
    const bool fwd_invalid = hdr_r > a.list_cap || hdr_miss != 0u || hdr_ovf != 0u;
    const int radius = __float_as_int(h.rec1.w);
    const bool touched = bwd_touched(h.s0, h.s1, h.s2x);
    const bool rendered = !fwd_invalid && radius > 0;
    if (!rendered || !(touched || a.dense)) {
        bwd_zero_row<STORE_SH>(a, idx, stage, rendered, radius);
        return;
    }
    bwd_full_row<STORE_SH, SH>(a, idx, h, cam, stage);
}

template <bool STORE_SH, int SH>
__global__ void __launch_bounds__(256, SGR_PRE_BWD_BLOCKS) k_preprocess_bwd(PreprocessBwdArgs a)
{
    __shared__ float s_stage[STORE_SH ? 4 * 48 * 65 : 1];
    const bool staged = STORE_SH && a.M == 16 && (((uintptr_t)a.dL_dsh) & 15) == 0;
    const int lane = threadIdx.x & 63, wave = threadIdx.x >> 6;
    float* panel = s_stage + (STORE_SH ? wave * (48 * 65) : 0);
    preprocess_bwd_lane<STORE_SH, SH>(a, staged ? panel + lane : nullptr, blockIdx.x * 256 + threadIdx.x);
    if (STORE_SH && staged) {
        __builtin_amdgcn_fence(__ATOMIC_ACQ_REL, "wavefront");
        __builtin_amdgcn_wave_barrier();
        const long long row0 = (long long)blockIdx.x * 256 + wave * 64;
        const int rows = (int)min(64ll, (long long)a.P - row0);
        float4* out4 = reinterpret_cast<float4*>(a.dL_dsh + (size_t)(row0 > 0 ? row0 : 0) * 48);
#pragma unroll
        for (int it = 0; it < 12; it++) {
            const int j4 = it * 64 + lane;
            if (j4 < rows * 12) {
                const int row = j4 / 12, e0 = (j4 % 12) * 4;
                const float* src = panel + 65 * e0 + row;
                out4[j4] = make_float4(src[0], src[65], src[130], src[195]);
            }
        }
    }
}

__global__ void __launch_bounds__(256) k_masked_colors(int P, const GeomRec* __restrict__ rec, const float* __restrict__ acc,
                                                       float* __restrict__ out, const float* __restrict__ cam_pos,
                                                       float* __restrict__ campos_row)
{
    const int idx = blockIdx.x * 256 + threadIdx.x;
    if (campos_row && idx < 3) campos_row[idx] = cam_pos[idx];
    if (idx >= P) return;
    const GeomRec* rp = rec + idx;
    const size_t i3 = 3 * (size_t)idx;
    if (!(rp->radius > 0)) { out[i3] = 0.f; out[i3 + 1] = 0.f; out[i3 + 2] = 0.f; return; }
    const uint32_t clamped = rp->clamped;
    const float4 s0 = *reinterpret_cast<const float4*>(acc + SGR_ACC_STRIDE * (size_t)idx);
    out[i3] = (clamped & 1u) ? 0.f : s0.x;
    out[i3 + 1] = (clamped & 2u) ? 0.f : s0.y;
    out[i3 + 2] = (clamped & 4u) ? 0.f : s0.z;
}

__device__ __forceinline__ void sh_dir_sum_over_views(int idx, size_t P, int V, int D, const float* __restrict__ means3D,
                                                      const float* __restrict__ campos, const float* __restrict__ dcolor,
                                                      const float* row, float* dm)
{
    const size_t i3 = 3 * (size_t)idx;
    const float mx = means3D[i3], my = means3D[i3 + 1], mz = means3D[i3 + 2];
    dm[0] = 0.f; dm[1] = 0.f; dm[2] = 0.f;
    for (int v = 0; v < V; v++) {
        const float* g = dcolor + ((size_t)v * P + idx) * 3;
        const float g0 = g[0], g1 = g[1], g2 = g[2];
        if (g0 == 0.f && g1 == 0.f && g2 == 0.f) continue;
        const float dx = mx - campos[3 * v], dy = my - campos[3 * v + 1], dz = mz - campos[3 * v + 2];
        const float len = sqrtf(dx * dx + dy * dy + dz * dz);
        const float x = dx / len, y = dy / len, z = dz / len;
        float dL_ddir[3] = {0.f, 0.f, 0.f};
#pragma unroll 1
        for (int c = 0; c < 3; c++) {
            float h[16];
#pragma unroll
            for (int k = 0; k < 16; k++) h[k] = row[3 * k + c];
            const float dL_dRGB = (c == 0 ? g0 : (c == 1 ? g1 : g2)) * 1.0f;
            float dRGBdx, dRGBdy, dRGBdz;
            sh_dir_channel(D, h, x, y, z, dRGBdx, dRGBdy, dRGBdz);
            dL_ddir[0] += dRGBdx * dL_dRGB; dL_ddir[1] += dRGBdy * dL_dRGB; dL_ddir[2] += dRGBdz * dL_dRGB;
        }
        const float sum2 = dx * dx + dy * dy + dz * dz;
        const float invsum32 = 1.0f / sqrtf(sum2 * sum2 * sum2);
        dm[0] += ((+sum2 - dx * dx) * dL_ddir[0] - dy * dx * dL_ddir[1] - dz * dx * dL_ddir[2]) * invsum32;
        dm[1] += (-dx * dy * dL_ddir[0] + (sum2 - dy * dy) * dL_ddir[1] - dz * dy * dL_ddir[2]) * invsum32;
        dm[2] += (-dx * dz * dL_ddir[0] - dy * dz * dL_ddir[1] + (sum2 - dz * dz) * dL_ddir[2]) * invsum32;
    }
}

__device__ __forceinline__ void sh_grad_sum_over_views(int idx, size_t P, int V, int D, const float* __restrict__ means3D,
                                                       const float* __restrict__ campos, const float* __restrict__ dcolor,
                                                       float* acc)
{
    const size_t i3 = 3 * (size_t)idx;
    const float mx = means3D[i3], my = means3D[i3 + 1], mz = means3D[i3 + 2];
#pragma unroll
    for (int k = 0; k < 48; k++) acc[k] = 0.f;
    for (int v = 0; v < V; v++) {
        const float* g = dcolor + ((size_t)v * P + idx) * 3;
        const float g0 = g[0], g1 = g[1], g2 = g[2];
        if (g0 == 0.f && g1 == 0.f && g2 == 0.f) continue;
        float dx = mx - campos[3 * v], dy = my - campos[3 * v + 1], dz = mz - campos[3 * v + 2];
        const float len = sqrtf(dx * dx + dy * dy + dz * dz);
        const float x = dx / len, y = dy / len, z = dz / len;
        float b[16];
        b[0] = SH_C0;
        if (D > 0) {
            b[1] = -SH_C1 * y; b[2] = SH_C1 * z; b[3] = -SH_C1 * x;
            if (D > 1) {
                const float xx = x * x, yy = y * y, zz = z * z, xy = x * y, yz = y * z, xz = x * z;
                b[4] = SH_C2[0] * xy; b[5] = SH_C2[1] * yz; b[6] = SH_C2[2] * (2.f * zz - xx - yy);
                b[7] = SH_C2[3] * xz; b[8] = SH_C2[4] * (xx - yy);
                if (D > 2) {
                    b[9] = SH_C3[0] * y * (3.f * xx - yy); b[10] = SH_C3[1] * xy * z;
                    b[11] = SH_C3[2] * y * (4.f * zz - xx - yy); b[12] = SH_C3[3] * z * (2.f * zz - 3.f * xx - 3.f * yy);
                    b[13] = SH_C3[4] * x * (4.f * zz - xx - yy); b[14] = SH_C3[5] * z * (xx - yy);
                    b[15] = SH_C3[6] * x * (xx - 3.f * yy);
                }
            }
        }
// ... 221 lines not shown
    const int idx = blockIdx.x * 256 + threadIdx.x;
    if (idx >= a.P) return;
    float x, y, z, vx, vy, vz, len;
    sh_rgb_dir(a, idx, x, y, z, vx, vy, vz, len);
    float sh[48];
    load_sh_n(a.sh, idx, a.M, a.n, sh);
    const size_t i3 = 3 * (size_t)idx;
    colors[i3] = fmax_(sh_channel(a.D, sh, 0, x, y, z), 0.0f);
    colors[i3 + 1] = fmax_(sh_channel(a.D, sh, 1, x, y, z), 0.0f);
    colors[i3 + 2] = fmax_(sh_channel(a.D, sh, 2, x, y, z), 0.0f);
}

__global__ void __launch_bounds__(256) k_sh_to_rgb_bwd(ShRgbArgs a, const float* __restrict__ dL_dcolors,
                                                       float* __restrict__ dL_dsh, float* __restrict__ dL_dpositions,
                                                       float* __restrict__ dL_ddirections)
{
    const int idx = blockIdx.x * 256 + threadIdx.x;
    if (idx >= a.P) return;
    float x, y, z, vx, vy, vz, len;
    sh_rgb_dir(a, idx, x, y, z, vx, vy, vz, len);
    float sh[48], dsh[48];
    load_sh_n(a.sh, idx, a.M, a.n, sh);
#pragma unroll
    for (int k = 0; k < 48; k++) dsh[k] = 0.0f;
    const size_t i3 = 3 * (size_t)idx;
    const float dcol[3] = {dL_dcolors[i3], dL_dcolors[i3 + 1], dL_dcolors[i3 + 2]};
    const uint32_t clamped = (sh_channel(a.D, sh, 0, x, y, z) < 0.f ? 1u : 0u) | (sh_channel(a.D, sh, 1, x, y, z) < 0.f ? 2u : 0u) |
                             (sh_channel(a.D, sh, 2, x, y, z) < 0.f ? 4u : 0u);
    float dL_ddir[3] = {0, 0, 0};
    sh_backward(a.D, sh, dcol, clamped, x, y, z, dsh, dL_ddir);
    if (dL_dsh) {
        float* dst = dL_dsh + (size_t)idx * a.M * 3;
        const int n_sh = 3 * a.M;
        if (n_sh == 48 && ((uintptr_t)dst & 15) == 0) {
            float4* d4 = reinterpret_cast<float4*>(dst);
#pragma unroll
            for (int i = 0; i < 12; i++) { float4 o = {dsh[4 * i], dsh[4 * i + 1], dsh[4 * i + 2], dsh[4 * i + 3]}; d4[i] = o; }
        } else {
#pragma unroll
            for (int i = 0; i < 48; i++) if (i < n_sh) dst[i] = dsh[i];
        }
    }
    if (a.positions) {
        if (dL_dpositions) {
            const float dot = x * dL_ddir[0] + y * dL_ddir[1] + z * dL_ddir[2];
            const float inv = 1.0f / len;
            dL_dpositions[i3] = (dL_ddir[0] - x * dot) * inv;
            dL_dpositions[i3 + 1] = (dL_ddir[1] - y * dot) * inv;
            dL_dpositions[i3 + 2] = (dL_ddir[2] - z * dot) * inv;
        }
    } else if (dL_ddirections) {
        dL_ddirections[i3] = dL_ddir[0]; dL_ddirections[i3 + 1] = dL_ddir[1]; dL_ddirections[i3 + 2] = dL_ddir[2];
    }
}

}

void sgr_launch_mark_visible(int P, const float* means3D, const float* viewmatrix, uint8_t* present, hipStream_t s)
{
    if (P <= 0) return;
    hipLaunchKernelGGL(k_mark_visible, dim3((P + 255) / 256), dim3(256), 0, s, P, means3D, viewmatrix, present);
}

void sgr_launch_depth_keys(const PreprocessArgs& a, hipStream_t s)
{
    if (a.P <= 0) return;
    hipLaunchKernelGGL(k_depth_keys, dim3((a.P + 255) / 256), dim3(256), 0, s, a);
}

void sgr_launch_preprocess_fwd(const PreprocessArgs& a, hipStream_t s)
{
    if (a.P <= 0) return;
    const dim3 grid((a.P + 255) / 256);
    if (a.colors_precomp) hipLaunchKernelGGL(k_preprocess_fwd<2>, grid, dim3(256), 0, s, a);
    else if (sh_fast_layout(a.shs, a.M)) hipLaunchKernelGGL(k_preprocess_fwd<0>, grid, dim3(256), 0, s, a);
    else hipLaunchKernelGGL(k_preprocess_fwd<1>, grid, dim3(256), 0, s, a);
}

void sgr_launch_preprocess_bwd(const PreprocessBwdArgs& a, hipStream_t s)
{
    if (a.P <= 0) return;
    const dim3 grid((a.P + 255) / 256);
    const int mode = (!a.shs || a.sh_dir_elsewhere) ? 2 : (sh_fast_layout(a.shs, a.M) ? 0 : 1);
    if (a.dL_dsh) {
        if (mode == 0) hipLaunchKernelGGL((k_preprocess_bwd<true, 0>), grid, dim3(256), 0, s, a);
        else if (mode == 1) hipLaunchKernelGGL((k_preprocess_bwd<true, 1>), grid, dim3(256), 0, s, a);
        else hipLaunchKernelGGL((k_preprocess_bwd<true, 2>), grid, dim3(256), 0, s, a);
    } else {
        if (mode == 0) hipLaunchKernelGGL((k_preprocess_bwd<false, 0>), grid, dim3(256), 0, s, a);
        else if (mode == 1) hipLaunchKernelGGL((k_preprocess_bwd<false, 1>), grid, dim3(256), 0, s, a);
        else hipLaunchKernelGGL((k_preprocess_bwd<false, 2>), grid, dim3(256), 0, s, a);
    }
}

void sgr_launch_masked_colors(int P, const GeomRec* rec, const float* acc, float* out, const float* cam_pos, float* campos_row,
                              hipStream_t s)
{
    hipLaunchKernelGGL(k_masked_colors, dim3((P + 255) / 256), dim3(256), 0, s, P, rec, acc, out, cam_pos, campos_row);
}

void sgr_launch_sh_adam_from_views(int P, int V, int D, int M, size_t vstride, const float* means3D, const float* campos,
                                   const float* dcolor, float* sh, float* exp_avg, float* exp_avg_sq, float lr_dc, float lr_rest, float b1, float b2,
                                   float eps, float bc1, float bc2_sqrt, float grad_scale, float* dmean_extra, hipStream_t s,
                                   const uint32_t* guard, uint32_t guard_cap, uint8_t* reach)
{
    ShAdamArgs a = {lr_dc, lr_rest, b1, b2, sgr_one_minus(b1), sgr_one_minus(b2), eps, bc1, bc2_sqrt, grad_scale, guard, guard_cap, reach};
    if (reach)
        hipLaunchKernelGGL((k_sh_adam_from_views<false, true>), dim3((P + 63) / 64), dim3(64), 0, s, P, V, D, M, vstride, means3D, campos,
                           dcolor, sh, exp_avg, exp_avg_sq, a, dmean_extra);
    else if (dmean_extra)
        hipLaunchKernelGGL(k_sh_adam_from_views<true>, dim3((P + 63) / 64), dim3(64), 0, s, P, V, D, M, vstride, means3D, campos, dcolor,
                           sh, exp_avg, exp_avg_sq, a, dmean_extra);
    else
        hipLaunchKernelGGL(k_sh_adam_from_views<false>, dim3((P + 63) / 64), dim3(64), 0, s, P, V, D, M, vstride, means3D, campos, dcolor,
                           sh, exp_avg, exp_avg_sq, a, dmean_extra);
}

void sgr_launch_sh_adam_zero(const SgrShAdamJob& job, hipStream_t s)
{
    if (job.P <= 0) return;
    hipLaunchKernelGGL(k_sh_adam_zero, dim3((job.P + 63) / 64), dim3(64), 0, s, job);
}

void sgr_launch_sh_grad_from_views(int P, int V, int D, int M, size_t vstride, const float* means3D, const float* campos,
                                   const float* dcolor, float* dL_dsh, hipStream_t s)
{
    hipLaunchKernelGGL(k_sh_grad_from_views, dim3((P + 255) / 256), dim3(256), 0, s, P, V, D, M, vstride, means3D, campos, dcolor,
                       dL_dsh);
}

static int sh_rgb_args(ShRgbArgs& a, int P, int D, int M, const float* sh, const float* positions, const float* centers,
                       int n_centers, const float* directions)
{
    if (D < 0 || D > 3 || M < (D + 1) * (D + 1) || M > 16 || !sh) return SGR_E_INVALID;
    if (positions ? (!centers || (n_centers != 1 && n_centers != P)) : !directions) return SGR_E_INVALID;
    a.P = P; a.D = D; a.M = M; a.n = (D + 1) * (D + 1); a.sh = sh; a.positions = positions; a.centers = centers;
    a.n_centers = n_centers; a.directions = directions;
    return 0;
}

extern "C" int sgr_sh_to_rgb_forward(int P, int D, int M, const float* sh, const float* positions, const float* camera_centers,
                                     int n_centers, const float* directions, float* colors, void* stream)
{
    if (P <= 0) return 0;
    ShRgbArgs a;
    if (!colors || sh_rgb_args(a, P, D, M, sh, positions, camera_centers, n_centers, directions) < 0) return SGR_E_INVALID;
    hipLaunchKernelGGL(k_sh_to_rgb_fwd, dim3((P + 255) / 256), dim3(256), 0, (hipStream_t)stream, a, colors);
    return sgr_launch_status();
}

extern "C" int sgr_sh_to_rgb_backward(int P, int D, int M, const float* sh, const float* positions, const float* camera_centers,
                                      int n_centers, const float* directions, const float* dL_dcolors, float* dL_dsh,
                                      float* dL_dpositions, float* dL_ddirections, void* stream)
{
    if (P <= 0) return 0;
    ShRgbArgs a;
    if (!dL_dcolors || sh_rgb_args(a, P, D, M, sh, positions, camera_centers, n_centers, directions) < 0) return SGR_E_INVALID;
    hipLaunchKernelGGL(k_sh_to_rgb_bwd, dim3((P + 255) / 256), dim3(256), 0, (hipStream_t)stream, a, dL_dcolors, dL_dsh,
                       dL_dpositions, dL_ddirections);
    return sgr_launch_status();
}
```

### sugar_amd/csrc/sgr_common.h

```cpp
#pragma once
#include <cmath>
#include <cstdio>
#include <cstdlib>
#include <hip/hip_runtime.h>
#include <stdint.h>
#include <stddef.h>
#include "../../include/sugar_raster.h"

#define SGR_TILE_X 16
#define SGR_TILE_Y 16
#define SGR_TILE_PIX 256
#define SGR_NUM_CUS 256
#define SGR_LEGACY_LDS_BYTES (150 * 1024)
#define SGR_BIN_SLICES 1024

struct GeomRec {
    float x, y, cx, cy;
    float cz, opacity, depth;
    int radius;
    float r, g, b;
    uint32_t clamped;
};
static_assert(sizeof(GeomRec) == 48, "GeomRec must be 48 bytes");

int sgr_fail(int code, const char* msg);
static inline int sgr_launch_status() { return hipGetLastError() == hipSuccess ? 0 : SGR_E_HIP; }

static inline size_t sgr_align(size_t x, size_t a = 256) { return (x + a - 1) / a * a; }
static inline size_t sgr_geom_acc_offset(int P) { return sgr_align((size_t)(P > 0 ? P : 1) * 48); }
size_t sgr_sort_scratch_bytes(int P);
#define SGR_ACC_STRIDE 16
static inline size_t sgr_geom_sort_offset(int P) { return sgr_geom_acc_offset(P) + sgr_align((size_t)(P > 0 ? P : 1) * SGR_ACC_STRIDE * 4); }
size_t sgr_sort_rects_offset(int P);
hipError_t sgr_acc_reset(char* geom_buffer, int P, hipStream_t s);
static inline size_t sgr_geom_reach_offset(int P) { return sgr_geom_sort_offset(P) + sgr_align(sgr_sort_scratch_bytes(P)); }
static inline size_t sgr_geom_total(int P) { return sgr_geom_reach_offset(P) + sgr_align((size_t)(P > 0 ? P : 1)); }

struct ImgLayout {
    size_t final_T, n_contrib, tile_start, tile_cursor, tile_maxc, tile_walked, blk_nb, header, repair_flag, repair_list, deep_list, blk_hist, total;
    int n_blocks;
    int gx, gy, T;
};
static inline ImgLayout sgr_img_layout(int W, int H)
{
    ImgLayout L;
    L.gx = (W + SGR_TILE_X - 1) / SGR_TILE_X;
    L.gy = (H + SGR_TILE_Y - 1) / SGR_TILE_Y;
    L.T = L.gx * L.gy;
    size_t off = 0;
    L.final_T = off;     off = sgr_align(off + (size_t)W * H * 4);
    L.n_contrib = off;   off = sgr_align(off + (size_t)W * H * 4);
    L.tile_start = off;  off = sgr_align(off + (size_t)(L.T + 1) * 4);
    L.tile_cursor = off; off = sgr_align(off + (size_t)L.T * 4);
    L.tile_maxc = off;   off = sgr_align(off + (size_t)L.T * 4);
    L.tile_walked = off; off = sgr_align(off + (size_t)L.T * 4);
    L.blk_nb = off;      off = sgr_align(off + (size_t)L.T * 16);
    L.header = off;      off = sgr_align(off + 64);
    L.repair_flag = off; off = sgr_align(off + (size_t)L.T * 4);
    L.repair_list = off; off = sgr_align(off + (size_t)L.T * 4);
    L.deep_list = off;   off = sgr_align(off + (size_t)L.T * 4);
    L.n_blocks = ((size_t)L.T * 4 <= SGR_LEGACY_LDS_BYTES) ? SGR_BIN_SLICES : 0;
    L.blk_hist = off;    off = sgr_align(off + (size_t)L.n_blocks * L.T * 4);
    L.total = off;
    return L;
}
#define SGR_SUP 8
#define SGR_SUP_SHIFT 3
#ifndef SGR_B2_SLICES
#define SGR_B2_SLICES 2048
#endif
#define SGR_B2_CHUNK 512
#define SGR_B2_HDR_R1 0
#define SGR_B2_HDR_CHUNKS 1
#define SGR_B2_HDR_OVERFLOW 2
struct Bin2Layout {
    size_t hist1, sup_count, sup_start, chunk_base, hdr, L1, cnt2, chunk_sup, total;
    int sgx, sgy, T1, per_slice;
    uint32_t cap1, chunk_cap;
};
Bin2Layout sgr_bin2_layout(int P, int gx, int gy);
void sgr_launch_bin2_count(int P, int gx, int gy, const Bin2Layout& L, char* scratch, uint32_t* hdr, const uint2* rects,
                           const uint32_t* order, uint32_t* tile_count, uint32_t chunk_grid, hipStream_t s);
void sgr_launch_bin2_write(int gx, int gy, const Bin2Layout& L, char* scratch, const uint32_t* hdr, uint32_t n_chunks, const uint2* rects,
                           const uint32_t* order, const uint32_t* tile_start, uint32_t* point_list, uint32_t list_cap,
                           const uint32_t* tile_need, hipStream_t s, const uint32_t* gate = nullptr, uint32_t max_grid = 0u);

struct BinLayout { size_t point_list, blk_mask, total; };
#define SGR_BIN_MASK_OFFSET(cap) ((((size_t)(cap) * 4 + 255) / 256) * 256)
static inline BinLayout sgr_bin_layout(int64_t R, int T)
{
    BinLayout L;
    size_t off = 0;
    L.point_list = off; off = sgr_align(off + (size_t)R * 4);
    L.blk_mask = off;   off = sgr_align(off + ((size_t)(R >> 6) + (size_t)T + 2) * 32);
    L.total = off < 256 ? 256 : off;
    return L;
}


enum { SGR_STAGE_PREPROCESS = 0, SGR_STAGE_SCAN , SGR_STAGE_SCATTER, SGR_STAGE_SORT , SGR_STAGE_BLEND_FWD,
       SGR_STAGE_BLEND_BWD, SGR_STAGE_PREPROCESS_BWD, SGR_STAGE_HINT_REPAIR ,
       SGR_STAGE_FWD_POST , SGR_STAGE_LOSS_FWD, SGR_STAGE_LOSS_BWD,
       SGR_STAGE_FILL , SGR_STAGE_SH_ADAM, SGR_STAGE_ADAM, SGR_STAGE_MASKED_COLORS, SGR_STAGE_COUNT };
struct SgrStageTimer {
    hipStream_t s; int stage; hipEvent_t a = nullptr, b = nullptr; bool live = false;
    SgrStageTimer(hipStream_t s_, int stage_);
    void stop();
    ~SgrStageTimer() { stop(); }
};

struct PreprocessArgs {
    int P, D, M;
    const float* means3D; const float* scales; float scale_modifier; const float* rotations;
    const float* opacities; const float* shs; const float* cov3D_precomp; const float* colors_precomp;
    const float* viewmatrix; const float* projmatrix; const float* cam_pos;
    int W, H; float tan_fovx, tan_fovy, focal_x, focal_y;
    int gx, gy;
    int* radii; GeomRec* rec;
    int raw_params;
    uint32_t* sort_keys;
    uint2* rect_by_id;
    uint2* key_minmax;
    uint32_t* sort_counters; int n_sort_counters;
    int keys_elsewhere = 0;
    uint32_t* zero_words = nullptr; int n_zero_words = 0;
};
void sgr_launch_mark_visible(int P, const float* means3D, const float* viewmatrix, uint8_t* present, hipStream_t s);
void sgr_launch_preprocess_fwd(const PreprocessArgs& a, hipStream_t s);
void sgr_launch_depth_keys(const PreprocessArgs& a, hipStream_t s);

struct PreprocessBwdArgs {
    int P, D, M;
    const float* means3D; const float* shs; const float* scales; const float* rotations; float scale_modifier;
    const float* cov3D_precomp; const float* viewmatrix; const float* projmatrix; const float* cam_pos;
    int W, H; float tan_fovx, tan_fovy, focal_x, focal_y;
    const GeomRec* rec;
    int raw_params;
    int sh_dir_elsewhere;
    float* campos_row;
    float* dens_max_radii; float* dens_accum; float* dens_denom;
    const uint32_t* header; uint32_t list_cap;
    float* acc;
    int acc_clean;
    int dense;
    float* dL_dmean2D; float* dL_dconic; float* dL_dopacity; float* dL_dcolor;
    float* dL_dmean3D; float* dL_dcov3D; float* dL_dsh; float* dL_dscale; float* dL_drot;
};
void sgr_launch_preprocess_bwd(const PreprocessBwdArgs& a, hipStream_t s);
void sgr_launch_masked_colors(int P, const GeomRec* rec, const float* acc, float* out, const float* cam_pos, float* campos_row, hipStream_t s);
void sgr_launch_sh_grad_from_views(int P, int V, int D, int M, size_t vstride, const float* means3D, const float* campos,
                                   const float* dcolor, float* dL_dsh, hipStream_t s);

static inline double sgr_intended_double(float x)
{
    static thread_local float memo_x[2] = {0.f, 0.f};
    static thread_local double memo_d[2] = {0.0, 0.0};
    for (int k = 0; k < 2; k++) if (memo_x[k] == x && memo_x[k] != 0.f) return memo_d[k];
    double out = (double)x;
    char buf[48];
    for (int p = 1; p <= 9; p++) {
        snprintf(buf, sizeof buf, "%.*g", p, (double)x);
        const double d = strtod(buf, nullptr);
        if ((float)d == x) { out = d; break; }
    }
    memo_x[1] = memo_x[0]; memo_d[1] = memo_d[0]; memo_x[0] = x; memo_d[0] = out;
    return out;
}
static inline float sgr_one_minus(float beta) { return (float)(1.0 - sgr_intended_double(beta)); }
static inline void sgr_bias_corrections(float beta1, float beta2, int step, float* bc1, float* bc2_sqrt)
{
    *bc1 = (float)(1.0 - pow(sgr_intended_double(beta1), (double)step));
    *bc2_sqrt = (float)sqrt(1.0 - pow(sgr_intended_double(beta2), (double)step));
}

void sgr_launch_sh_adam_from_views(int P, int V, int D, int M, size_t vstride, const float* means3D, const float* campos,
                                   const float* dcolor, float* sh, float* exp_avg, float* exp_avg_sq, float lr_dc, float lr_rest, float b1, float b2,
                                   float eps, float bc1, float bc2_sqrt, float grad_scale, float* dmean_extra, hipStream_t s,
                                   const uint32_t* guard = nullptr, uint32_t guard_cap = 0, uint8_t* reach = nullptr);
struct SgrShAdamJob {
    int P;
    int k;
    int n_groups, n_with;
    float* sh; float* exp_avg; float* exp_avg_sq;
    const uint8_t* reach;
    float lr_dc, lr_rest, b1, b2, omb1, omb2, eps, bc1, bc2_sqrt, grad_scale;
    float zero;
    const uint32_t* guard; uint32_t guard_cap;
};
void sgr_launch_sh_adam_zero(const SgrShAdamJob& job, hipStream_t s);
#define SGR_ADAM_OVERLAP_DEFAULT 1
int sgr_adam_overlap();
int sgr_adam_overlap_k();
int sgr_adam_launch(long long n, float* params, const float* grads, float* exp_avg, float* exp_avg_sq, int n_seg,
                    const long long* seg_begin, const long long* seg_end, const float* seg_lr_a, const float* seg_lr_b,
                    const int* seg_period, const int* seg_split, float beta1, float beta2, float eps, int step, float grad_scale,
                    const float* extra, long long extra_n, const uint32_t* guard, uint32_t guard_cap, hipStream_t s);

void sgr_launch_gaussian_sort(int P, char* sort_scratch, const uint32_t** order_out, const uint2* rect_by_id, uint2* rects_sorted,
                              hipStream_t s, int part = 0);
size_t sgr_sort_rect_by_id_offset(int P);
size_t sgr_sort_minmax_offset(int P);
size_t sgr_sort_counters_offset(int P);
int sgr_sort_counter_words();
void sgr_launch_bin_count(int P, int gx, int gy, int n_slices, int per_slice, const uint32_t* order, const uint2* rects,
                          uint32_t* blk_hist, hipStream_t s);
void sgr_launch_bin_scatter(int P, int gx, int gy, int n_slices, int per_slice, const uint32_t* order, const uint2* rects,
                            const uint32_t* tile_start, uint32_t* blk_hist, uint32_t* point_list, hipStream_t s);
void sgr_launch_hist_scan(int T, int n_blocks, uint32_t* blk_hist, uint32_t* tile_count, hipStream_t s);
void sgr_launch_tile_scan(int T, const uint32_t* tile_count, uint32_t* tile_start, uint32_t* header, uint32_t* tile_maxc,
                          uint32_t* tile_walked, int clear_b2_words, uint32_t* host_a, uint32_t* host_b, hipStream_t s,
                          uint32_t* repair_flag = nullptr);

void sgr_launch_blend_fwd(int W, int H, int gx, int gy, const uint32_t* tile_start, const uint32_t* point_list,
                          const GeomRec* rec, const float* bg, float* final_T, uint32_t* n_contrib, uint32_t* tile_maxc,
                          uint32_t* tile_walked, float* out_color, unsigned long long* blk_mask, uint32_t* blk_nb,
                          uint32_t* header, uint32_t list_cap, const uint32_t* tile_need, const uint32_t* launch_order, hipStream_t s,
                          uint32_t* repair_flag = nullptr, uint32_t* repair_list = nullptr, int exact = 0, uint32_t deep_min = 0u,
                          uint8_t* reach = nullptr);
void sgr_launch_deep_list(int gx, int gy, const uint32_t* tile_start, const uint32_t* tile_need, uint32_t deep_min, uint32_t* header,
                          uint32_t list_cap, uint32_t* deep_list, hipStream_t s);
void sgr_launch_blend_fwd_deep(int W, int H, int gx, int gy, const uint32_t* tile_start, const uint32_t* point_list, const GeomRec* rec,
                               const float* bg, float* final_T, uint32_t* n_contrib, uint32_t* tile_maxc, uint32_t* tile_walked,
                               float* out_color, unsigned long long* blk_mask, uint32_t* blk_nb, uint32_t* header, uint32_t list_cap,
                               const uint32_t* tile_need, uint32_t* deep_list, uint32_t deep_min, hipStream_t s, uint32_t* repair_flag,
                               uint32_t* repair_list, int exact);
int sgr_exact_alpha();
uint32_t sgr_deep_min();
#define SGR_REPAIR_TILES 1024
void sgr_launch_blend_fwd_repair(int W, int H, int gx, int gy, const uint32_t* tile_start, const uint32_t* point_list,
                                 const GeomRec* rec, const float* bg, float* final_T, uint32_t* n_contrib, uint32_t* tile_maxc,
                                 uint32_t* tile_walked, float* out_color, unsigned long long* blk_mask, uint32_t* blk_nb,
                                 uint32_t* header, uint32_t list_cap, const uint32_t* repair_list, hipStream_t s, int exact = 0,
                                 uint8_t* reach = nullptr);
void sgr_launch_blend_fwd_post(int gx, int gy, const uint32_t* tile_maxc, const uint32_t* tile_walked, uint32_t* header, uint32_t list_cap,
                               uint32_t* tile_need_out, float hint_margin, uint32_t* header_host_dev, uint32_t* order_scratch,
                               uint32_t* order_out, hipStream_t s);
void sgr_launch_blend_bwd(int W, int H, int gx, int gy, const uint32_t* tile_start, const uint32_t* point_list,
                          const char* binning, const uint32_t* blk_nb, const GeomRec* rec, const float* bg,
                          const float* final_T, const uint32_t* n_contrib, const float* dL_dpix, float* acc,
                          const uint32_t* tile_maxc, const uint32_t* header, uint32_t list_cap, uint32_t* tile_order, int order_ready,
                          hipStream_t s, int exact = 0, const SgrShAdamJob* job = nullptr);
int sgr_backward_job(int phase, int P, int D, int M, int64_t R, const float* background, int width, int height, const float* means3D,
                     const float* shs, const float* scales, const float* rotations, const float* viewmatrix, const float* projmatrix,
                     const float* cam_pos, float tan_fovx, float tan_fovy, char* geom_buffer, char* binning_buffer, char* img_buffer,
                     const float* dL_dpix, float* dL_dmean2D, float* dL_dopacity, float* dL_dcolor, float* dL_dmean3D, float* dL_dscale,
                     float* dL_drot, void* stream, const sgr_backward_opts* opts, const SgrShAdamJob* job);
struct SgrTileOrderJob;
extern "C" int sgr_l1_ssim_forward_job(int channels, int width, int height, const float* img, const float* gt, float lambda, char* scratch,
                                       float* loss_out, const SgrTileOrderJob* job, void* stream);
extern "C" int sgr_forward_post_job(int width, int height, char* img_buffer, int64_t R, const sgr_forward_opts* opts, SgrTileOrderJob* job);
#define SGR_FORWARD_INVALID(hdr, cap) ((hdr)[SGR_HDR_R] > (cap) || (hdr)[SGR_HDR_HINT_MISS] != 0u || (hdr)[4 + SGR_B2_HDR_OVERFLOW] != 0u)
```

### sugar_amd/csrc/train.hip

```cpp
#include "../../include/sugar_raster.h"
#include "sgr_common.h"
#include "tile_order.h"

#include <chrono>
#include <cmath>
#include <cstdlib>
#include <cstring>
#include <dlfcn.h>
#include <string>

namespace {

struct FixedBuf { char* p; size_t bytes; size_t asked; };
char* fixed_alloc(void* user, size_t bytes)
{
    FixedBuf* b = static_cast<FixedBuf*>(user);
    b->asked = bytes;
    return bytes <= b->bytes ? b->p : nullptr;
}

struct RcclUniqueId { char internal[128]; };
typedef void* RcclComm;
struct Rccl {
    void* handle = nullptr;
    int (*GetUniqueId)(RcclUniqueId*) = nullptr;
    int (*CommInitRank)(RcclComm*, int, RcclUniqueId, int) = nullptr;
    int (*CommDestroy)(RcclComm) = nullptr;
    int (*CommAbort)(RcclComm) = nullptr;
    int (*AllGather)(const void*, void*, size_t, int, RcclComm, hipStream_t) = nullptr;
    int (*AllReduce)(const void*, void*, size_t, int, int, RcclComm, hipStream_t) = nullptr;
    const char* (*GetErrorString)(int) = nullptr;
    bool ok() const { return GetUniqueId && CommInitRank && CommDestroy && AllGather && AllReduce; }
};
const int RCCL_FLOAT = 7, RCCL_SUM = 0;
Rccl& rccl()
{
    static Rccl r;
    if (r.handle) return r;
    for (const char* name : {"librccl.so.1", "librccl.so"}) {
        r.handle = dlopen(name, RTLD_NOW | RTLD_NOLOAD);
        if (r.handle) break;
    }
    if (!r.handle)
        for (const char* name : {"librccl.so.1", "librccl.so", "/opt/rocm/lib/librccl.so.1"}) {
            r.handle = dlopen(name, RTLD_NOW | RTLD_GLOBAL);
            if (r.handle) break;
        }
    if (!r.handle) return r;
    r.GetUniqueId = reinterpret_cast<decltype(r.GetUniqueId)>(dlsym(r.handle, "ncclGetUniqueId"));
    r.CommInitRank = reinterpret_cast<decltype(r.CommInitRank)>(dlsym(r.handle, "ncclCommInitRank"));
    r.CommDestroy = reinterpret_cast<decltype(r.CommDestroy)>(dlsym(r.handle, "ncclCommDestroy"));
    r.CommAbort = reinterpret_cast<decltype(r.CommAbort)>(dlsym(r.handle, "ncclCommAbort"));
    r.AllGather = reinterpret_cast<decltype(r.AllGather)>(dlsym(r.handle, "ncclAllGather"));
    r.AllReduce = reinterpret_cast<decltype(r.AllReduce)>(dlsym(r.handle, "ncclAllReduce"));
    r.GetErrorString = reinterpret_cast<decltype(r.GetErrorString)>(dlsym(r.handle, "ncclGetErrorString"));
    return r;
}

}

struct sgr_trainer {
    sgr_train_config c;
    RcclComm comm = nullptr;
    int world = 1, rank = 0;
    hipStream_t comm_stream = nullptr;
    hipEvent_t ev_colors = nullptr, ev_small = nullptr;
    int chunks = 1;
    hipEvent_t ev_gathered[16] = {}, ev_reduced[16] = {};
    float* recv = nullptr;
    float* campos_all = nullptr;
    double last_wait_ms = 0.0;
    hipEvent_t hdr_event = nullptr;
    bool have_forward = false;
    bool acc_dirty = true;
    bool defer_post = false;
    int64_t R = 0;
    long long seg_begin[4], seg_end[4];
    float seg_lr[4];
    int seg_one[4];
    std::string err;
};

extern "C" {

static thread_local std::string g_train_err;
static int tfail(int code, const std::string& m) { g_train_err = m; return code; }
const char* sgr_trainer_last_error(void) { return g_train_err.c_str(); }

sgr_trainer* sgr_trainer_create(const sgr_train_config* cfg)
{
    if (!cfg) { g_train_err = "null config"; return nullptr; }
    const sgr_train_config& c = *cfg;
    const bool ok = c.P > 0 && c.width > 0 && c.height > 0 && c.M >= (c.D + 1) * (c.D + 1) && c.M <= 16 && c.D >= 0 && c.D <= 3 &&
                    c.flat && c.flat_grad && c.exp_avg && c.exp_avg_sq && c.background && c.geom && c.img && c.binning &&
                    c.loss_scratch && c.image && c.grad_image && c.loss_out && c.colors && c.header_host &&
                    c.binning_capacity > 0 && c.n_small > 0 && (c.n_small & 3) == 0 && (c.off_features & 3) == 0;
    if (!ok) { g_train_err = "sgr_trainer_create: bad configuration (null pointer, size or alignment)"; return nullptr; }
    if (c.geom_bytes < sgr_geom_bytes(c.P) || c.img_bytes < sgr_img_bytes(c.width, c.height) + sgr_bin2_bytes(c.P, c.width, c.height) ||
        c.binning_bytes < sgr_binning_bytes(c.binning_capacity, c.width, c.height)) {
        g_train_err = "sgr_trainer_create: a scratch buffer is smaller than sgr_geom_bytes / sgr_img_bytes + sgr_bin2_bytes / sgr_binning_bytes";
        return nullptr;
    }
    sgr_trainer* t = new sgr_trainer;
    t->c = c;
    if (hipEventCreateWithFlags(&t->hdr_event, hipEventDisableTiming) != hipSuccess) { delete t; g_train_err = "hipEventCreate failed"; return nullptr; }
    const long long P = c.P;
    const long long b[4] = {c.off_xyz, c.off_opacity, c.off_scaling, c.off_rotation};
    const long long n[4] = {3 * P, P, 3 * P, 4 * P};
    const float lr[4] = {c.lr_xyz, c.lr_opacity, c.lr_scaling, c.lr_rotation};
    for (int k = 0; k < 4; k++) { t->seg_begin[k] = b[k]; t->seg_end[k] = b[k] + n[k]; t->seg_lr[k] = lr[k]; t->seg_one[k] = 1; }
    std::memset(c.header_host, 0, 64);
    if (hipMemset(c.geom + sgr_geom_reach_offset(c.P), 0, (size_t)c.P) != hipSuccess) {
        (void)hipEventDestroy(t->hdr_event); delete t; g_train_err = "sgr_trainer_create: clearing the reach flags failed"; return nullptr;
    }
    {
        void* mapped = nullptr;
        t->defer_post = hipHostGetDevicePointer(&mapped, c.header_host, 0) == hipSuccess && mapped && !getenv("SGR_TRAINER_NO_DEFER");
        if (!t->defer_post) (void)hipGetLastError();
    }
    return t;
}

void sgr_trainer_destroy(sgr_trainer* t)
{
    if (!t) return;
    (void)sgr_trainer_comm_destroy(t);
    if (t->hdr_event) (void)hipEventDestroy(t->hdr_event);
    delete t;
}

int sgr_trainer_set_binning(sgr_trainer* t, char* binning, size_t bytes, int64_t capacity)
{
    if (!t || !binning || capacity <= 0 || bytes < sgr_binning_bytes(capacity, t->c.width, t->c.height))
        return tfail(SGR_E_INVALID, "sgr_trainer_set_binning: bad buffer");
    t->c.binning = binning; t->c.binning_bytes = bytes; t->c.binning_capacity = capacity;
    return 0;
}

int sgr_trainer_acc_dirty(sgr_trainer* t) { return (t && !t->acc_dirty) ? 0 : 1; }

int sgr_trainer_forward_valid(sgr_trainer* t, uint32_t* header_out)
{
    if (!t || !t->have_forward) return tfail(SGR_E_INVALID, "sgr_trainer_forward_valid: no forward yet");
    if (hipEventSynchronize(t->hdr_event) != hipSuccess) return tfail(SGR_E_HIP, "hipEventSynchronize failed");
    const uint32_t* h = t->c.header_host;
    if (header_out) std::memcpy(header_out, h, 64);
    const bool bad = (int64_t)h[SGR_HDR_R] > t->R || h[8 + SGR_HDR_HINT_MISS] != 0u || h[SGR_HDR_L1_OVERFLOW] != 0u;
    return bad ? 0 : 1;
}

int sgr_trainer_step(sgr_trainer* t, const sgr_train_view* v, int phases, const sgr_train_exchange* ex, void* stream)
{
    if (!t || !v) return tfail(SGR_E_INVALID, "sgr_trainer_step: null argument");
    const sgr_train_config& c = t->c;
    hipStream_t s = (hipStream_t)stream;
    const int P = c.P, W = c.width, H = c.height;
    float* flat = c.flat;
    float* grad = c.flat_grad;
    const float* means3D = flat + c.off_xyz;
    const float* shs = flat + c.off_features;
    const float* opac = flat + c.off_opacity;
    const float* scal = flat + c.off_scaling;
    const float* rot = flat + c.off_rotation;
    const uint32_t* header = reinterpret_cast<const uint32_t*>(c.img + sgr_img_header_offset(W, H));
    const uint32_t cap = (uint32_t)(c.binning_capacity > 0xFFFFFFFFll ? 0xFFFFFFFFll : c.binning_capacity);
    const char* dense_env = getenv("SGR_BWD_DENSE");
    const bool bwd_dense = dense_env && dense_env[0] && dense_env[0] != '0';
    const int overlap = sgr_adam_overlap();
    const bool reach_ok = overlap != 0 && phases == 15 && !(v->flags & SGR_VIEW_DEEP_LISTS) && ex && ex->n_views == 1 && !ex->all_colors && !ex->all_campos &&
                          !(ex->g_end > ex->g_begin) && c.M == 16 && !bwd_dense &&
                          ((((uintptr_t)(flat + c.off_features) | (uintptr_t)(c.exp_avg + c.off_features) |
                             (uintptr_t)(c.exp_avg_sq + c.off_features)) & 15) == 0);
    const bool split = reach_ok && overlap == 1;
    uint8_t* reach = reinterpret_cast<uint8_t*>(c.geom + sgr_geom_reach_offset(P));
    if (phases & 1) {
        if (!v->viewmatrix || !v->projmatrix || !v->campos || !v->gt_image) return tfail(SGR_E_INVALID, "sgr_trainer_step: null view");
        FixedBuf g = {c.geom, c.geom_bytes, 0}, b = {c.binning, c.binning_bytes, 0}, i = {c.img, c.img_bytes, 0};
        sgr_forward_opts fo;
        std::memset(&fo, 0, sizeof(fo));
        fo.binning_capacity = c.binning_capacity;
        fo.flags = SGR_FLAG_RAW_PARAMS | ((v->flags & SGR_VIEW_DEEP_LISTS) ? 0 : SGR_FLAG_NO_DEEP) | (reach_ok ? SGR_FLAG_REACH : 0);
        fo.header_host = c.header_host;
        if (t->defer_post) fo.flags |= SGR_FLAG_DEFER_POST;
        fo.header_event = t->defer_post ? nullptr : t->hdr_event;
        fo.tile_need = v->tile_need;
        fo.tile_need_out = v->tile_need_out;
        fo.hint_margin = v->hint_margin;
        fo.chunk_grid = v->chunk_grid;
        fo.tile_order = v->tile_order;
        fo.tile_order_out = v->tile_order_out;
        const int64_t R = sgr_forward_ex(fixed_alloc, &g, fixed_alloc, &b, fixed_alloc, &i, P, c.D, c.M, c.background, W, H, means3D, shs,
                                         nullptr, opac, scal, 1.0f, rot, nullptr, v->viewmatrix, v->projmatrix, v->campos,
                                         v->tan_fovx, v->tan_fovy, 0, c.image, c.radii, 0, stream, &fo);
        if (R < 0) return tfail((int)R, std::string("forward: ") + sgr_last_error());
        t->R = R;
        t->have_forward = true;
        SgrTileOrderJob job = {};
        int rc = t->defer_post ? sgr_forward_post_job(W, H, c.img, R, &fo, &job) : 0;
        if (rc < 0) return tfail(rc, "sgr_forward_post_job failed");
        { SgrStageTimer tm(s, SGR_STAGE_LOSS_FWD); rc = sgr_l1_ssim_forward_job(3, W, H, c.image, v->gt_image, c.lambda_dssim, c.loss_scratch, nullptr, t->defer_post ? &job : nullptr, stream); }
        if (rc < 0) return tfail(rc, "l1_ssim_forward failed");
        if (t->defer_post && hipEventRecord(t->hdr_event, s) != hipSuccess) return tfail(SGR_E_HIP, "hipEventRecord failed");
        { SgrStageTimer tm(s, SGR_STAGE_LOSS_BWD); rc = sgr_l1_ssim_backward_ex(3, W, H, c.image, v->gt_image, c.lambda_dssim, c.loss_scratch, nullptr, c.grad_image, c.loss_out, stream); }
        if (rc < 0) return tfail(rc, "l1_ssim_backward failed");
    }
    if (phases & 3) {
        if (!t->have_forward) return tfail(SGR_E_INVALID, "sgr_trainer_step: backward before any forward");
        sgr_backward_opts bo = {c.max_radii2D, c.grad_accum, c.denom, c.colors + 3 * (size_t)P,
                                ((t->defer_post || v->tile_order_out) ? SGR_BWD_TILE_ORDER_READY : 0) | SGR_BWD_ACC_CLEAN |
                                    (bwd_dense ? SGR_BWD_DENSE : 0)};
        SgrShAdamJob job = {};
        if (split) {
            if (ex->step < 1) return tfail(SGR_E_INVALID, "sgr_trainer_step: exchange description missing");
            job.P = P; job.k = sgr_adam_overlap_k();
            job.sh = flat + c.off_features; job.exp_avg = c.exp_avg + c.off_features; job.exp_avg_sq = c.exp_avg_sq + c.off_features;
            job.reach = reach;
            job.lr_dc = c.lr_features_dc; job.lr_rest = c.lr_features_rest; job.b1 = c.beta1; job.b2 = c.beta2;
            job.omb1 = sgr_one_minus(c.beta1); job.omb2 = sgr_one_minus(c.beta2); job.eps = c.eps; job.grad_scale = ex->grad_scale;
            job.zero = 0.f; job.guard = header; job.guard_cap = cap;
            sgr_bias_corrections(c.beta1, c.beta2, ex->step, &job.bc1, &job.bc2_sqrt);
        }
        const int first = (phases & 3) == 3 ? 0 : ((phases & 1) ? 1 : 2);
        const int last = (phases & 3) == 3 ? 0 : ((phases & 2) ? 2 : 1);
        for (int ph = first; ph <= last; ph++) {
            if (ph != 2) {
                if (t->acc_dirty && sgr_acc_reset(c.geom, P, s) != hipSuccess)
                    return tfail(SGR_E_HIP, "sgr_trainer_step: accumulator reset failed");
                t->acc_dirty = true;
            }
            const int rc = sgr_backward_job(ph | SGR_MODE_RAW_PARAMS, P, c.D, c.M, t->R, c.background, W, H, means3D, shs, scal, rot,
                                            v->viewmatrix, v->projmatrix, v->campos, v->tan_fovx, v->tan_fovy, c.geom, c.binning, c.img,
                                            c.grad_image, c.dL_dmean2D, grad + c.off_opacity, c.colors, grad + c.off_xyz,
                                            grad + c.off_scaling, grad + c.off_rotation, stream, &bo, split ? &job : nullptr);
            if (rc < 0) return tfail(rc, std::string("backward: ") + sgr_last_error());
            if (ph != 1) t->acc_dirty = false;
        }
    }
    if (phases & 12) {
        if (!ex || ex->step < 1 || ex->n_views < 1) return tfail(SGR_E_INVALID, "sgr_trainer_step: exchange description missing");
        float bc1, bc2_sqrt;
        sgr_bias_corrections(c.beta1, c.beta2, ex->step, &bc1, &bc2_sqrt);
        if (phases & 4) {
            const float* cols = ex->all_colors ? ex->all_colors : c.colors;
            const float* cams = ex->all_campos ? ex->all_campos : (ex->all_colors ? nullptr : c.colors + 3 * (size_t)P);
            if (!cams) return tfail(SGR_E_INVALID, "sgr_trainer_step: all_campos missing");
            const size_t stride = (size_t)(ex->view_stride ? ex->view_stride : (ex->all_colors ? P : P + 1));
            const bool part = ex->g_end > ex->g_begin;
            const long long g0 = part ? ex->g_begin : 0, g1 = part ? ex->g_end : P;
            if (g0 < 0 || g1 > P || (g0 & 63)) return tfail(SGR_E_INVALID, "sgr_trainer_step: bad Gaussian range (g_begin must be a multiple of 64)");
            if (part && !ex->all_colors) cols += 3 * (size_t)g0;
            const size_t fo = (size_t)g0 * 3 * (size_t)c.M;
            SgrStageTimer tm(s, SGR_STAGE_SH_ADAM);
            sgr_launch_sh_adam_from_views((int)(g1 - g0), ex->n_views, c.D, c.M, stride, means3D + 3 * (size_t)g0, cams, cols,
                                          flat + c.off_features + fo, c.exp_avg + c.off_features + fo, c.exp_avg_sq + c.off_features + fo,
                                          c.lr_features_dc, c.lr_features_rest, c.beta1, c.beta2, c.eps, bc1, bc2_sqrt, ex->grad_scale, nullptr, s,
                                          header, cap, split ? reach : nullptr);
            tm.stop();
            if (hipGetLastError() != hipSuccess) return tfail(SGR_E_HIP, "sh_adam launch failed");
        }
        if (phases & 8) {
            const bool part = ex->f_end > ex->f_begin;
            const long long f0 = part ? ex->f_begin : 0, f1 = part ? ex->f_end : c.n_small;
            if (f0 < 0 || f1 > c.n_small || (f0 & 3)) return tfail(SGR_E_INVALID, "sgr_trainer_step: bad float range (f_begin must be a multiple of 4)");
            long long sb[4], se[4];
            for (int k = 0; k < 4; k++) { sb[k] = t->seg_begin[k] - f0; se[k] = t->seg_end[k] - f0; }
            SgrStageTimer tm(s, SGR_STAGE_ADAM);
            const int rc = sgr_adam_launch(f1 - f0, flat + f0, grad + f0, c.exp_avg + f0, c.exp_avg_sq + f0, 4, sb, se, t->seg_lr, t->seg_lr,
                                           t->seg_one, t->seg_one, c.beta1, c.beta2, c.eps, ex->step, ex->grad_scale, nullptr, 0, header,
                                           cap, s);
            tm.stop();
            if (rc < 0) return tfail(rc, "adam launch failed");
        }
    }
    return 0;
}


int sgr_rccl_unique_id(char* out128)
{
    Rccl& r = rccl();
    if (!r.ok()) return tfail(SGR_E_INVALID, "RCCL could not be loaded (librccl.so)");
    RcclUniqueId id;
    const int rc = r.GetUniqueId(&id);
    if (rc != 0) return tfail(SGR_E_HIP, std::string("ncclGetUniqueId: ") + (r.GetErrorString ? r.GetErrorString(rc) : "failed"));
    std::memcpy(out128, id.internal, 128);
    return 0;
}

int sgr_trainer_comm_init(sgr_trainer* t, const char* id128, int world, int rank, float* recv, size_t recv_bytes)
{
    if (!t || !id128 || world < 1 || rank < 0 || rank >= world || !recv) return tfail(SGR_E_INVALID, "sgr_trainer_comm_init: bad argument");
    if (recv_bytes < (size_t)world * ((size_t)t->c.P + 1) * 3 * sizeof(float))
        return tfail(SGR_E_INVALID, "sgr_trainer_comm_init: receive buffer smaller than world x (P + 1) x 3 floats");
    if (t->comm) return tfail(SGR_E_INVALID, "sgr_trainer_comm_init: already initialised");
    Rccl& r = rccl();
    if (!r.ok()) return tfail(SGR_E_INVALID, "RCCL could not be loaded (librccl.so)");
    RcclUniqueId id;
    std::memcpy(id.internal, id128, 128);
    int rc = r.CommInitRank(&t->comm, world, id, rank);
    if (rc != 0) { t->comm = nullptr; return tfail(SGR_E_HIP, std::string("ncclCommInitRank: ") + (r.GetErrorString ? r.GetErrorString(rc) : "failed")); }
    t->world = world; t->rank = rank; t->recv = recv;
    bool ok = hipStreamCreateWithFlags(&t->comm_stream, hipStreamNonBlocking) == hipSuccess;
    for (hipEvent_t* e : {&t->ev_colors, &t->ev_small})
        ok = ok && hipEventCreateWithFlags(e, hipEventDisableTiming) == hipSuccess;
    for (int k = 0; k < 16; k++)
        ok = ok && hipEventCreateWithFlags(&t->ev_gathered[k], hipEventDisableTiming) == hipSuccess &&
             hipEventCreateWithFlags(&t->ev_reduced[k], hipEventDisableTiming) == hipSuccess;
    ok = ok && hipMalloc(reinterpret_cast<void**>(&t->campos_all), (size_t)world * 3 * sizeof(float)) == hipSuccess;
    if (!ok) { (void)sgr_trainer_comm_destroy(t); return tfail(SGR_E_HIP, "sgr_trainer_comm_init: stream / event / buffer creation failed"); }
    return 0;
}

int sgr_trainer_comm_abort(sgr_trainer* t)
{
    if (!t || !t->comm) return 0;
    Rccl& r = rccl();
    if (r.CommAbort) (void)r.CommAbort(t->comm); else (void)r.CommDestroy(t->comm);
    t->comm = nullptr;
// ... 104 lines not shown
```

### sugar_amd/train_step.py

```python
from __future__ import annotations

from math import exp

import torch
import torch.distributed as dist
import torch.nn.functional as F

from ._call import call, ptr


def l1_loss(network_output, gt):
    return torch.abs((network_output - gt)).mean()


def _gaussian(window_size, sigma):
    gauss = torch.Tensor([exp(-(x - window_size // 2) ** 2 / float(2 * sigma ** 2)) for x in range(window_size)])
    return gauss / gauss.sum()


_WINDOWS: dict = {}


def create_window(window_size, channel, like: torch.Tensor):
    key = (window_size, channel, like.device, like.dtype)
# ... 447 lines not shown
        self._hdr = torch.zeros(16, dtype=torch.int32).pin_memory()
        self._deep_min = int(lib.sgr_get_deep_min()) or (1 << 31)
        self._last_max_need = 0
        self._hints = {}
        self._pending = None
        self.redone = 0
        self.last_num_rendered = 0
        self.repaired_tiles, self.last_repaired_tiles = 0, 0
        self.T = ((self.W + 15) // 16) * ((self.H + 15) // 16)
        self._h = None
        self._allocate()
        explicit = native_collectives is True
        if native_collectives is None:
            env = _os.environ.get("SGR_NATIVE_COLLECTIVES")
            native_collectives = (env == "1") if env is not None else (self.exchange and self.world > 1 and dist.get_backend() == "nccl")
        self.native_collectives = False
        if native_collectives and self.exchange:
            if dist.get_backend() != "nccl":
                raise RuntimeError("native_collectives needs the RCCL (\"nccl\") process group backend")
            idbuf = C.create_string_buffer(128)
            have_id = 1 if (dist.get_rank() != 0 or lib.sgr_rccl_unique_id(idbuf) >= 0) else 0
            box = [idbuf.raw, have_id]
            dist.broadcast_object_list(box, src=0)
            ok, why = bool(box[1]), "sgr_rccl_unique_id failed on rank 0"
            if ok:
                with torch.cuda.device(dev):
                    rc = lib.sgr_trainer_comm_init(self._h, box[0], self.world, dist.get_rank(), self._recv.data_ptr(), self._recv.numel() * 4)
                ok = rc >= 0
                if not ok:
                    why = "sgr_trainer_comm_init failed: " + lib.sgr_trainer_last_error().decode(errors="replace")
            flag = torch.tensor([1 if ok else 0], dtype=torch.int32, device=dev)
            dist.all_reduce(flag, op=dist.ReduceOp.MIN)
            if int(flag.item()) == 1:
                self.native_collectives = True
                lib.sgr_trainer_set_exchange_chunks(self._h, self.exchange_chunks)
            else:
                if ok:
                    lib.sgr_trainer_comm_destroy(self._h)
                    why = "another rank could not initialise its communicator"
                if explicit:
                    raise RuntimeError("native_collectives: " + why)
                import warnings
                warnings.warn("in-library gradient exchange unavailable (" + why + "): using torch.distributed collectives")

    def set_exchange_chunks(self, n: int):
        n = int(n)
        if not 1 <= n <= 16:
            raise ValueError("exchange chunks: 1 .. 16")
        self.exchange_chunks = n
        if getattr(self, "native_collectives", False) and self._lib.sgr_trainer_set_exchange_chunks(self._h, n) < 0:
            raise RuntimeError("sgr_trainer_set_exchange_chunks failed")

    def _allocate(self):
        C, lib, _lib, params, dev = self._C, self._lib, self._L, self.params, self.dev
        P, M = params.P, params.M
        u8 = lambda n: torch.empty(int(n), dtype=torch.uint8, device=dev)
        self._geom = u8(lib.sgr_geom_bytes(P))
        self._img = u8(lib.sgr_img_bytes(self.W, self.H) + lib.sgr_bin2_bytes(P, self.W, self.H))
        self._binning = u8(lib.sgr_binning_bytes(self.capacity, self.W, self.H))
        self._loss_scratch = u8(lib.sgr_l1_ssim_scratch_bytes(3, self.W, self.H))
        self.image = torch.empty(3, self.H, self.W, device=dev)
        self._grad_image = torch.empty(3, self.H, self.W, device=dev)
        self.loss_out = torch.zeros(3, device=dev)
        self._send = torch.zeros(P + 1, 3, device=dev)
        self._recv = torch.empty(self.world * (P + 1), 3, device=dev) if self.exchange else None
        self._cams_all = torch.empty(self.world, 3, device=dev) if self.exchange else None
        self.radii = torch.zeros(P, dtype=torch.int32, device=dev)
        if self.densify_stats:
            self.viewspace_grad = torch.zeros(P, 3, device=dev)
            self.max_radii2D = torch.zeros(P, device=dev)
            self.xyz_gradient_accum = torch.zeros(P, device=dev)
            self.denom = torch.zeros(P, device=dev)
        o, vp = params.offsets, (lambda t: t.data_ptr() if t is not None else None)
        st = (lambda name: vp(getattr(self, name))) if self.densify_stats else (lambda name: None)
        betas = self._betas
        self._cfg = _lib.TrainConfig(
            P, self.sh_degree, M, self.W, self.H, vp(params.flat), vp(params.flat_grad), vp(self.exp_avg), vp(self.exp_avg_sq),
            o["xyz"], o["opacity"], o["scaling"], o["rotation"], o["features"], params.n_small,
            params.LRS["xyz"], params.LRS["opacity"], params.LRS["scaling"], params.LRS["rotation"], params.LRS["features"],
            params.REST_LR, betas[0], betas[1], self._eps, self._lambda_dssim, vp(self.bg), vp(self._geom), self._geom.numel(),
            vp(self._img), self._img.numel(), vp(self._binning), self._binning.numel(), self.capacity, vp(self._loss_scratch),
            vp(self.image), vp(self._grad_image), vp(self.loss_out), vp(self._send), vp(self.radii), vp(self._hdr),
            st("viewspace_grad"), st("max_radii2D"), st("xyz_gradient_accum"), st("denom"))
        self._h = lib.sgr_trainer_create(C.byref(self._cfg))
        if not self._h:
            raise RuntimeError("sgr_trainer_create failed: " + lib.sgr_trainer_last_error().decode(errors="replace"))

    def all_reduce_densification_stats(self, group=None):
        if not self.densify_stats:
            raise RuntimeError("all_reduce_densification_stats: the trainer was built without densify_stats=True")
        self.synchronize()
        from .view_parallel import all_reduce_densification_stats
        all_reduce_densification_stats(self, group=group)

    def densify_and_prune(self, max_grad=0.0002, min_opacity=0.005, extent=1.0, max_screen_size=None, seed=None, group=None):
        from . import densify
        if self.world > 1 or (dist.is_available() and dist.is_initialized()):
            self.all_reduce_densification_stats(group)
        else:
            self.synchronize()
        if seed is not None or getattr(self, "_densify_gen", None) is None:
            self._densify_gen = torch.Generator(device=self.dev).manual_seed(int(seed or 0))
        g = self._densify_gen
        p = self.params
        stats = dict(xyz_gradient_accum=self.xyz_gradient_accum, denom=self.denom, max_radii2D=self.max_radii2D)
        t, m1, m2, nc, ns, npr = densify.densify_and_prune(p.raw(), p.split_flat(self.exp_avg), p.split_flat(self.exp_avg_sq), stats,
                                                           max_grad=max_grad, min_opacity=min_opacity, extent=extent,
                                                           max_screen_size=max_screen_size, generator=g)
        self.resize(t, m1, m2)
        return nc, ns, npr

    def resize(self, tensors, exp_avg=None, exp_avg_sq=None):
        self.synchronize()
        old_P = self.params.P
        if getattr(self, "native_collectives", False):
            raise RuntimeError("resize: not with the in-library exchange (its receive buffer is registered with the communicator)")
        if self._h:
            self._lib.sgr_trainer_destroy(self._h)
            self._h = None
        params = GaussianParams.from_raw(tensors, self.dev)
        self.params = params
        self.exp_avg = torch.zeros_like(params.flat)
        self.exp_avg_sq = torch.zeros_like(params.flat)
        with torch.no_grad():
            for buf, src in ((self.exp_avg, exp_avg), (self.exp_avg_sq, exp_avg_sq)):
                if src is not None:
                    for k, v in params.split_flat(buf).items():
                        v.copy_(src[k].reshape(v.shape))
        self.capacity = max(int(self.capacity * (params.P / max(old_P, 1)) * 1.1), 1 << 20)
        self._pending = None
        self._allocate()
        return params


    def __del__(self):
        try:
            if getattr(self, "_h", None):
                self._lib.sgr_trainer_destroy(self._h)
                self._h = None
        except Exception:
            pass

    def _call(self, cam, gt, key, phases, ex, use_hint=True, exchange_step=None):
        import time as _time
        _t0 = _time.perf_counter()
        C, L = self._C, self._L
        need = need_out = order = order_out = None
        if phases & 1:
            ent = self._hints.get(key)
            if ent is None:
                ent = self._hints[key] = [torch.zeros(self.T, dtype=torch.int32, device=self.dev), False, 0,
                                          torch.zeros(self.T, dtype=torch.int32, device=self.dev), False, 0]
            if self.walk_hint:
                need = ent[0].data_ptr() if (ent[1] and use_hint and self._calls >= self._hint_pause_until) else None
                need_out = ent[0].data_ptr()
            if self.launch_order:
                order = ent[3].data_ptr() if ent[4] else None
                order_out = ent[3].data_ptr()
            self._last_hinted = need is not None
            self._calls += 1
        ent5 = self._hints.get(key)
        deep = 1 if (need is not None and ent5 is not None and ent5[5] > self._deep_min) else 0
        view = L.TrainView(cam.viewmatrix.data_ptr(), cam.projmatrix.data_ptr(), cam.campos.data_ptr(), cam.tanfovx, cam.tanfovy,
                           gt.data_ptr(), need, need_out, self.hint_margin, self._chunk_grid(key), order, order_out, deep)
        with torch.cuda.device(self.dev):
            stream = C.c_void_p(torch.cuda.current_stream(self.dev).cuda_stream)
            if exchange_step is not None:
                rc = self._lib.sgr_trainer_step_exchange(self._h, C.byref(view), int(exchange_step), stream)
            else:
                rc = self._lib.sgr_trainer_step(self._h, C.byref(view), phases, C.byref(ex) if ex is not None else None, stream)
        self.host_work_s += _time.perf_counter() - _t0
        if exchange_step is not None:
            self.host_work_s -= 1e-3 * float(self._lib.sgr_trainer_last_exchange_wait_ms(self._h))
        if rc < 0:
            raise RuntimeError(f"sgr_trainer_step failed ({rc}): " + self._lib.sgr_trainer_last_error().decode(errors="replace"))
        return rc

    def _chunk_grid(self, key):
        ent = self._hints.get(key)
        n = ent[2] if ent is not None else 0
        return (n + n // 4 + 64) if n else 0

    def _grow(self, R):
        self.capacity = int(R) + int(R) // 2 + 65536
        self._binning = torch.empty(int(self._lib.sgr_binning_bytes(self.capacity, self.W, self.H)), dtype=torch.uint8, device=self.dev)
        rc = self._lib.sgr_trainer_set_binning(self._h, self._binning.data_ptr(), self._binning.numel(), self.capacity)
        if rc < 0:
            raise RuntimeError("sgr_trainer_set_binning failed")

    def _valid(self):
        hdr = (self._C.c_uint32 * 16)()
        ok = self._lib.sgr_trainer_forward_valid(self._h, hdr)
        if ok < 0:
            raise RuntimeError("sgr_trainer_forward_valid failed")
        self.last_num_rendered = int(hdr[0])
        self._last_chunks = int(hdr[5])
        self.last_repaired_tiles = int(hdr[8 + 7])
        self._last_max_need = int(hdr[8 + 1])
        if ok:
            self.repaired_tiles += self.last_repaired_tiles
        return bool(ok), (int(hdr[0]) if int(hdr[0]) > self.capacity else 0), bool(hdr[8 + 3])

    def _hint_feedback(self, missed):
        if missed:
            self._recent_misses = [t for t in self._recent_misses if t > self._calls - 32] + [self._calls]
            if len(self._recent_misses) >= 3:
                self._hint_pause_until = self._calls + 64
                self._recent_misses = []
                self.hint_pauses += 1

    def _repair(self, key, R, missed):
        self.redone += 1
        self._hint_feedback(missed)
        if R:
            torch.cuda.synchronize(self.dev)
            self._grow(R)
        if missed and key in self._hints:
            self._hints[key][1] = False

    def _resolve(self):
        while self._pending is not None:
            cam, gt, key = self._pending
            ok, R, missed = self._valid()
            if ok:
                if key in self._hints:
                    self._hints[key][1] = True
                    self._hints[key][2] = self._last_chunks
                    self._hints[key][4] = True
                    self._hints[key][5] = self._last_max_need
                self._hint_feedback(False)
                self._pending = None
                return
            if not (R or missed):
                raise RuntimeError("level-1 binning overflow: this view needs the single-level binning (use ViewShardedTrainer)")
            self._repair(key, R, missed)
            ex = self._L.TrainExchange(1, None, 0, None, 1.0, self.t)
            self._call(cam, gt, key, 15, ex)

    def step(self, cam, gt_image, cam_key=None):
        key = id(cam) if cam_key is None else cam_key
        if not self.exchange:
            self._resolve()
            self.t += 1
            ex = self._L.TrainExchange(1, None, 0, None, 1.0, self.t)
            self._call(cam, gt_image, key, 15, ex)
            self._pending = (cam, gt_image, key)
            return self.loss_out[0]
# ... 71 lines not shown
```

Before: 1061 images/s.

## Skip preprocess-backward work for unreached Gaussians using reach and row-dirty flags

Adds a per-Gaussian row-dirty byte array next to the reach flags, plus a packed preprocess-backward kernel. The kernel compacts reached rows into a shared list so wavefronts only process Gaussians the rasterizer touched. Unreached rows are zeroed only when they were written non-zero on an earlier step, which saves the gradient writes to already-zero rows. Correctness depends on tracking whether the gradient buffers changed outside the trainer, done here with tensor version stamps, a new invalidate API and a rows-unknown flag. Out-of-order lanes also disable the coalesced accumulator clear.

```diff
diff --git a/include/sugar_raster.h b/include/sugar_raster.h
--- a/include/sugar_raster.h
+++ b/include/sugar_raster.h
@@ -119,6 +119,8 @@
 #define SGR_BWD_TILE_ORDER_READY 1
 #define SGR_BWD_DENSE 8
 #define SGR_BWD_ACC_CLEAN 4
+#define SGR_BWD_ROWS_BY_REACH 16
+#define SGR_BWD_ROWS_UNKNOWN 32
 int sgr_backward_ex(int phase, int P, int D, int M, int64_t R,
                     const float* background, int width, int height,
                     const float* means3D, const float* shs, const float* colors_precomp,
@@ -154,6 +156,9 @@
 void sgr_set_adam_overlap(int on);
 int sgr_get_adam_overlap(void);
 size_t sgr_geom_reach_offset_bytes(int P);
+void sgr_set_rows_by_reach(int on);
+int sgr_get_rows_by_reach(void);
+size_t sgr_geom_rowdirty_offset_bytes(int P);
 
 int sgr_mark_visible(int P, const float* means3D, const float* viewmatrix, const float* projmatrix,
                      uint8_t* present, void* stream);
@@ -257,6 +262,7 @@
 int sgr_trainer_forward_valid(sgr_trainer* t, uint32_t* header_out);
 const char* sgr_trainer_last_error(void);
 int sgr_trainer_acc_dirty(sgr_trainer* t);
+void sgr_trainer_invalidate_rows(sgr_trainer* t);
 int sgr_rccl_unique_id(char* out128);
 int sgr_trainer_comm_init(sgr_trainer* t, const char* id128, int world, int rank, float* recv, size_t recv_bytes);
 int sgr_trainer_comm_destroy(sgr_trainer* t);
diff --git a/sugar_amd/_lib.py b/sugar_amd/_lib.py
--- a/sugar_amd/_lib.py
+++ b/sugar_amd/_lib.py
@@ -51,6 +51,10 @@
     "sgr_set_adam_overlap": (None, [_i]),
     "sgr_get_adam_overlap": (_i, []),
     "sgr_geom_reach_offset_bytes": (_sz, [_i]),
+    "sgr_set_rows_by_reach": (None, [_i]),
+    "sgr_trainer_invalidate_rows": (None, [_vp]),
+    "sgr_get_rows_by_reach": (_i, []),
+    "sgr_geom_rowdirty_offset_bytes": (_sz, [_i]),
     "sgr_geom_bytes": (_sz, [_i]),
     "sgr_img_bytes": (_sz, [_i, _i]),
     "sgr_binning_bytes": (_sz, [_i64, _i, _i]),
@@ -209,6 +213,7 @@
 
 SGR_FLAG_RAW_PARAMS, SGR_FLAG_SINGLE_LEVEL_BINNING, SGR_FLAG_SPECULATIVE = 1, 2, 8
 SGR_BWD_TILE_ORDER_READY, SGR_BWD_ACC_CLEAN, SGR_BWD_DENSE = 1, 4, 8
+SGR_BWD_ROWS_BY_REACH, SGR_BWD_ROWS_UNKNOWN = 16, 32
 HDR_R, HDR_HINT_MISS, HDR_L1_OVERFLOW = 0, 3, 6
 
 _lib = None
diff --git a/sugar_amd/csrc/capi.hip b/sugar_amd/csrc/capi.hip
--- a/sugar_amd/csrc/capi.hip
+++ b/sugar_amd/csrc/capi.hip
@@ -128,10 +128,19 @@
     if (k < 0) { const char* e = getenv("SGR_ADAM_OVERLAP_K"); k = e ? atoi(e) : 24; if (k < 8 || (k & 7)) k = 24; }
     return k;
 }
+static int g_rows_by_reach = -1;
+int sgr_rows_by_reach()
+{
+    if (g_rows_by_reach < 0) { const char* e = getenv("SGR_ROWS_BY_REACH"); g_rows_by_reach = (e && e[0] == '0') ? 0 : 1; }
+    return g_rows_by_reach;
+}
 
 extern "C" {
 
 int sgr_abi_version(void) { return SGR_ABI_VERSION; }
+void sgr_set_rows_by_reach(int on) { g_rows_by_reach = on ? 1 : 0; }
+int sgr_get_rows_by_reach(void) { return sgr_rows_by_reach(); }
+size_t sgr_geom_rowdirty_offset_bytes(int P) { return sgr_geom_rowdirty_offset(P); }
 void sgr_set_adam_overlap(int on) { g_adam_overlap = on == 2 ? 2 : (on ? 1 : 0); }
 int sgr_get_adam_overlap(void) { return sgr_adam_overlap(); }
 size_t sgr_geom_reach_offset_bytes(int P) { return sgr_geom_reach_offset(P); }
@@ -504,6 +513,9 @@
 
     float* acc = reinterpret_cast<float*>(geom_buffer + sgr_geom_acc_offset(P));
     const bool acc_clean = opts && (opts->flags & SGR_BWD_ACC_CLEAN);
+    const bool by_reach = opts && (opts->flags & SGR_BWD_ROWS_BY_REACH) && phase != 1;
+    if (by_reach && (dL_dsh || (opts->flags & SGR_BWD_DENSE)))
+        return fail(SGR_E_INVALID, "SGR_BWD_ROWS_BY_REACH is for a backward without dL_dsh and excludes SGR_BWD_DENSE");
     if (phase != 2) {
         if (!acc_clean) HIP_TRY(sgr_acc_reset(geom_buffer, P, s));
         if (R > 0) {
@@ -539,6 +551,9 @@
     pb.acc = acc;
     pb.acc_clean = acc_clean ? 1 : 0;
     pb.dense = (opts && (opts->flags & SGR_BWD_DENSE)) ? 1 : 0;
+    pb.reach = by_reach ? reinterpret_cast<const uint8_t*>(geom_buffer + sgr_geom_reach_offset(P)) : nullptr;
+    pb.rowdirty = by_reach ? reinterpret_cast<uint8_t*>(geom_buffer + sgr_geom_rowdirty_offset(P)) : nullptr;
+    pb.rows_unknown = (by_reach && (opts->flags & SGR_BWD_ROWS_UNKNOWN)) ? 1 : 0;
     pb.header = reinterpret_cast<const uint32_t*>(img_buffer + IL.header);
     pb.list_cap = (uint32_t)(R > 0xFFFFFFFFll ? 0xFFFFFFFFll : R);
     pb.campos_row = (opts && compact && phase == 0) ? opts->campos_row : nullptr;
diff --git a/sugar_amd/csrc/preprocess.hip b/sugar_amd/csrc/preprocess.hip
--- a/sugar_amd/csrc/preprocess.hip
+++ b/sugar_amd/csrc/preprocess.hip
@@ -441,6 +441,11 @@
     ap[0] = z4; ap[1] = z4;
     a.acc[SGR_ACC_STRIDE * (size_t)idx + 8] = 0.f;
 }
+__device__ __forceinline__ void bwd_zero_row_stats(const PreprocessBwdArgs& a, int idx, int radius)
+{
+    if (a.dens_denom) a.dens_denom[idx] += 1.0f;
+    if (a.dens_max_radii) a.dens_max_radii[idx] = fmaxf(a.dens_max_radii[idx], (float)radius);
+}
 template <bool STORE_SH>
 __device__ __forceinline__ void bwd_zero_row(const PreprocessBwdArgs& a, int idx, float* __restrict__ stage, bool stats, int radius)
 {
@@ -462,9 +467,19 @@
     }
     if (a.dL_dscale) { a.dL_dscale[i3] = 0; a.dL_dscale[i3 + 1] = 0; a.dL_dscale[i3 + 2] = 0; }
     if (a.dL_drot) { float4 z = {0, 0, 0, 0}; *reinterpret_cast<float4*>(a.dL_drot + 4 * (size_t)idx) = z; }
-    if (stats) {
-        if (a.dens_denom) a.dens_denom[idx] += 1.0f;
-        if (a.dens_max_radii) a.dens_max_radii[idx] = fmaxf(a.dens_max_radii[idx], (float)radius);
+    if (stats) bwd_zero_row_stats(a, idx, radius);
+}
+
+__device__ __forceinline__ void bwd_unreached_row(const PreprocessBwdArgs& a, int idx, bool row_dirty, bool fwd_invalid)
+{
+    int radius = 0;
+    if ((a.dens_denom || a.dens_max_radii) && !fwd_invalid) radius = a.rec[idx].radius;
+    const bool rendered = radius > 0;
+    if (row_dirty) {
+        bwd_zero_row<false>(a, idx, nullptr, rendered, radius);
+        a.rowdirty[idx] = 0;
+    } else if (rendered) {
+        bwd_zero_row_stats(a, idx, radius);
     }
 }
 
@@ -699,22 +714,40 @@
 }
 
 template <bool STORE_SH, int SH>
-__device__ __forceinline__ void preprocess_bwd_lane(const PreprocessBwdArgs& a, float* __restrict__ stage, const int idx0)
+__device__ __forceinline__ void preprocess_bwd_lane(const PreprocessBwdArgs& a, float* __restrict__ stage, const int idx0,
+                                                    const bool consecutive = true)
 {
     if (a.campos_row && idx0 < 3) a.campos_row[idx0] = a.cam_pos[idx0];
     uint32_t hdr_r = 0u, hdr_miss = 0u, hdr_ovf = 0u;
     if (a.header) { hdr_r = a.header[SGR_HDR_R]; hdr_miss = a.header[SGR_HDR_HINT_MISS]; hdr_ovf = a.header[4 + SGR_B2_HDR_OVERFLOW]; }
     const bool valid = idx0 < a.P;
     const int idx = valid ? idx0 : a.P - 1;
+    const bool by_reach = !STORE_SH && a.reach != nullptr;
+    bool reached = true, row_dirty = true;
+    if (by_reach) {
+        const uint8_t f = a.reach[idx], d = a.rowdirty[idx];
+        reached = valid && f != 0;
+        row_dirty = a.rows_unknown || d != 0;
+        if (!__any(reached)) {
+            if (valid) bwd_unreached_row(a, idx, row_dirty, hdr_r > a.list_cap || hdr_miss != 0u || hdr_ovf != 0u);
+            return;
+        }
+    }
     const float cam_raw = cam_request(a.viewmatrix, a.projmatrix, a.cam_pos);
     BwdHead h;
-    bwd_head_load(a, idx, h);
+    if (by_reach) {
+        const float4 z4 = {0.f, 0.f, 0.f, 0.f};
+        h.rec0 = z4; h.rec1 = z4; h.rec2 = z4; h.s0 = z4; h.s1 = z4; h.s2x = 0.f;
+        if (reached) bwd_head_load(a, idx, h);
+    } else {
+        bwd_head_load(a, idx, h);
+    }
     Cam cam;
     cam_unpack(cam_raw, cam);
     if (a.acc_clean) {
         const bool dirty = valid && bwd_touched(h.s0, h.s1, h.s2x);
         const unsigned long long m = __ballot(dirty);
-        if (__popcll(m) >= 32) {
+        if (consecutive && __popcll(m) >= 32) {
             const int lane = threadIdx.x & 63;
             const long long row0 = (long long)idx0 - lane;
             float4* w4 = reinterpret_cast<float4*>(a.acc + SGR_ACC_STRIDE * (size_t)row0);
@@ -730,10 +763,16 @@
     }
     if (!valid) return;
     const bool fwd_invalid = hdr_r > a.list_cap || hdr_miss != 0u || hdr_ovf != 0u;
+    if (by_reach && !reached) {
+        bwd_unreached_row(a, idx, row_dirty, fwd_invalid);
+        return;
+    }
     const int radius = __float_as_int(h.rec1.w);
     const bool touched = bwd_touched(h.s0, h.s1, h.s2x);
     const bool rendered = !fwd_invalid && radius > 0;
-    if (!rendered || !(touched || a.dense)) {
+    const bool full = rendered && (touched || a.dense);
+    if (by_reach && (a.rows_unknown || row_dirty != full)) a.rowdirty[idx] = full ? 1 : 0;
+    if (!full) {
         bwd_zero_row<STORE_SH>(a, idx, stage, rendered, radius);
         return;
     }
@@ -764,6 +803,53 @@
             }
         }
     }
+}
+
+template <int SH>
+__global__ void __launch_bounds__(256, SGR_PRE_BWD_BLOCKS) k_preprocess_bwd_packed(PreprocessBwdArgs a)
+{
+    __shared__ int s_list[256];
+    __shared__ int s_n;
+    const int tid = threadIdx.x, lane = tid & 63;
+    const long long base = (long long)blockIdx.x * 256;
+    const int rows = (int)min(256ll, (long long)a.P - base);
+    if (a.campos_row && blockIdx.x == 0 && tid < 3) a.campos_row[tid] = a.cam_pos[tid];
+    if (tid < 64) {
+        uint32_t rw = 0u, dw = 0u;
+        if (4 * lane < rows) {
+            rw = *reinterpret_cast<const uint32_t*>(a.reach + base + 4 * lane);
+            dw = *reinterpret_cast<const uint32_t*>(a.rowdirty + base + 4 * lane);
+            const int live = rows - 4 * lane;
+            if (live < 4) { const uint32_t keep = (1u << (8 * live)) - 1u; rw &= keep; dw &= keep; }
+        }
+        unsigned long long m[4];
+        int n_reached = 0;
+#pragma unroll
+        for (int j = 0; j < 4; j++) { m[j] = __ballot(((rw >> (8 * j)) & 0xFFu) != 0u); n_reached += __popcll(m[j]); }
+        const bool in_order = 4 * n_reached >= 3 * rows || a.dens_denom || a.dens_max_radii || a.rows_unknown;
+        if (!in_order) {
+            const unsigned long long below = (1ull << lane) - 1ull;
+            int at = 0;
+#pragma unroll
+            for (int j = 0; j < 4; j++) {
+                const int g = (int)base + 4 * lane + j;
+                if ((rw >> (8 * j)) & 0xFFu) {
+                    s_list[at + __popcll(m[j] & below)] = g;
+                } else if (((dw >> (8 * j)) & 0xFFu) != 0u) {
+                    bwd_unreached_row(a, g, true, false);
+                }
+                at += __popcll(m[j]);
+            }
+        }
+        if (lane == 0) s_n = in_order ? -1 : n_reached;
+    }
+    __syncthreads();
+    const int listed = s_n;
+    const bool in_order = listed < 0;
+    const int n = in_order ? rows : listed;
+    if ((tid & ~63) >= n) return;
+    const int idx0 = in_order ? (int)base + tid : (tid < n ? s_list[tid] : a.P);
+    preprocess_bwd_lane<false, SH>(a, nullptr, idx0, in_order);
 }
 
 __global__ void __launch_bounds__(256) k_masked_colors(int P, const GeomRec* __restrict__ rec, const float* __restrict__ acc,
@@ -1151,6 +1237,12 @@
     if (a.P <= 0) return;
     const dim3 grid((a.P + 255) / 256);
     const int mode = (!a.shs || a.sh_dir_elsewhere) ? 2 : (sh_fast_layout(a.shs, a.M) ? 0 : 1);
+    if (a.reach && !a.dL_dsh) {
+        if (mode == 0) hipLaunchKernelGGL((k_preprocess_bwd_packed<0>), grid, dim3(256), 0, s, a);
+        else if (mode == 1) hipLaunchKernelGGL((k_preprocess_bwd_packed<1>), grid, dim3(256), 0, s, a);
+        else hipLaunchKernelGGL((k_preprocess_bwd_packed<2>), grid, dim3(256), 0, s, a);
+        return;
+    }
     if (a.dL_dsh) {
         if (mode == 0) hipLaunchKernelGGL((k_preprocess_bwd<true, 0>), grid, dim3(256), 0, s, a);
         else if (mode == 1) hipLaunchKernelGGL((k_preprocess_bwd<true, 1>), grid, dim3(256), 0, s, a);
diff --git a/sugar_amd/csrc/sgr_common.h b/sugar_amd/csrc/sgr_common.h
--- a/sugar_amd/csrc/sgr_common.h
+++ b/sugar_amd/csrc/sgr_common.h
@@ -34,7 +34,8 @@
 size_t sgr_sort_rects_offset(int P);
 hipError_t sgr_acc_reset(char* geom_buffer, int P, hipStream_t s);
 static inline size_t sgr_geom_reach_offset(int P) { return sgr_geom_sort_offset(P) + sgr_align(sgr_sort_scratch_bytes(P)); }
-static inline size_t sgr_geom_total(int P) { return sgr_geom_reach_offset(P) + sgr_align((size_t)(P > 0 ? P : 1)); }
+static inline size_t sgr_geom_rowdirty_offset(int P) { return sgr_geom_reach_offset(P) + sgr_align((size_t)(P > 0 ? P : 1)); }
+static inline size_t sgr_geom_total(int P) { return sgr_geom_rowdirty_offset(P) + sgr_align((size_t)(P > 0 ? P : 1)); }
 
 struct ImgLayout {
     size_t final_T, n_contrib, tile_start, tile_cursor, tile_maxc, tile_walked, blk_nb, header, repair_flag, repair_list, deep_list, blk_hist, total;
@@ -143,6 +144,8 @@
     float* acc;
     int acc_clean;
     int dense;
+    const uint8_t* reach; uint8_t* rowdirty;
+    int rows_unknown;
     float* dL_dmean2D; float* dL_dconic; float* dL_dopacity; float* dL_dcolor;
     float* dL_dmean3D; float* dL_dcov3D; float* dL_dsh; float* dL_dscale; float* dL_drot;
 };
@@ -190,6 +193,7 @@
 void sgr_launch_sh_adam_zero(const SgrShAdamJob& job, hipStream_t s);
 #define SGR_ADAM_OVERLAP_DEFAULT 1
 int sgr_adam_overlap();
+int sgr_rows_by_reach();
 int sgr_adam_overlap_k();
 int sgr_adam_launch(long long n, float* params, const float* grads, float* exp_avg, float* exp_avg_sq, int n_seg,
                     const long long* seg_begin, const long long* seg_end, const float* seg_lr_a, const float* seg_lr_b,
diff --git a/sugar_amd/csrc/train.hip b/sugar_amd/csrc/train.hip
--- a/sugar_amd/csrc/train.hip
+++ b/sugar_amd/csrc/train.hip
@@ -73,6 +73,7 @@
     hipEvent_t hdr_event = nullptr;
     bool have_forward = false;
     bool acc_dirty = true;
+    bool rows_unknown = true;
     bool defer_post = false;
     int64_t R = 0;
     long long seg_begin[4], seg_end[4];
@@ -110,7 +111,7 @@
     const float lr[4] = {c.lr_xyz, c.lr_opacity, c.lr_scaling, c.lr_rotation};
     for (int k = 0; k < 4; k++) { t->seg_begin[k] = b[k]; t->seg_end[k] = b[k] + n[k]; t->seg_lr[k] = lr[k]; t->seg_one[k] = 1; }
     std::memset(c.header_host, 0, 64);
-    if (hipMemset(c.geom + sgr_geom_reach_offset(c.P), 0, (size_t)c.P) != hipSuccess) {
+    if (hipMemset(c.geom + sgr_geom_reach_offset(c.P), 0, sgr_geom_rowdirty_offset(c.P) + (size_t)c.P - sgr_geom_reach_offset(c.P)) != hipSuccess) {
         (void)hipEventDestroy(t->hdr_event); delete t; g_train_err = "sgr_trainer_create: clearing the reach flags failed"; return nullptr;
     }
     {
@@ -138,6 +139,7 @@
 }
 
 int sgr_trainer_acc_dirty(sgr_trainer* t) { return (t && !t->acc_dirty) ? 0 : 1; }
+void sgr_trainer_invalidate_rows(sgr_trainer* t) { if (t) t->rows_unknown = true; }
 
 int sgr_trainer_forward_valid(sgr_trainer* t, uint32_t* header_out)
 {
@@ -172,6 +174,7 @@
                           ((((uintptr_t)(flat + c.off_features) | (uintptr_t)(c.exp_avg + c.off_features) |
                              (uintptr_t)(c.exp_avg_sq + c.off_features)) & 15) == 0);
     const bool split = reach_ok && overlap == 1;
+    const bool by_reach = split && sgr_rows_by_reach() != 0;
     uint8_t* reach = reinterpret_cast<uint8_t*>(c.geom + sgr_geom_reach_offset(P));
     if (phases & 1) {
         if (!v->viewmatrix || !v->projmatrix || !v->campos || !v->gt_image) return tfail(SGR_E_INVALID, "sgr_trainer_step: null view");
@@ -208,7 +211,9 @@
         if (!t->have_forward) return tfail(SGR_E_INVALID, "sgr_trainer_step: backward before any forward");
         sgr_backward_opts bo = {c.max_radii2D, c.grad_accum, c.denom, c.colors + 3 * (size_t)P,
                                 ((t->defer_post || v->tile_order_out) ? SGR_BWD_TILE_ORDER_READY : 0) | SGR_BWD_ACC_CLEAN |
-                                    (bwd_dense ? SGR_BWD_DENSE : 0)};
+                                    (bwd_dense ? SGR_BWD_DENSE : 0) |
+                                    (by_reach ? (SGR_BWD_ROWS_BY_REACH | (t->rows_unknown ? SGR_BWD_ROWS_UNKNOWN : 0)) : 0)};
+        t->rows_unknown = true;
         SgrShAdamJob job = {};
         if (split) {
             if (ex->step < 1) return tfail(SGR_E_INVALID, "sgr_trainer_step: exchange description missing");
@@ -234,6 +239,7 @@
                                             grad + c.off_scaling, grad + c.off_rotation, stream, &bo, split ? &job : nullptr);
             if (rc < 0) return tfail(rc, std::string("backward: ") + sgr_last_error());
             if (ph != 1) t->acc_dirty = false;
+            if (by_reach) t->rows_unknown = false;
         }
     }
     if (phases & 12) {
diff --git a/sugar_amd/train_step.py b/sugar_amd/train_step.py
--- a/sugar_amd/train_step.py
+++ b/sugar_amd/train_step.py
@@ -553,6 +553,7 @@
             vp(self._img), self._img.numel(), vp(self._binning), self._binning.numel(), self.capacity, vp(self._loss_scratch),
             vp(self.image), vp(self._grad_image), vp(self.loss_out), vp(self._send), vp(self.radii), vp(self._hdr),
             st("viewspace_grad"), st("max_radii2D"), st("xyz_gradient_accum"), st("denom"))
+        self._rows_token, self._rows_stamp = object(), None
         self._h = lib.sgr_trainer_create(C.byref(self._cfg))
         if not self._h:
             raise RuntimeError("sgr_trainer_create failed: " + lib.sgr_trainer_last_error().decode(errors="replace"))
@@ -634,6 +635,13 @@
         deep = 1 if (need is not None and ent5 is not None and ent5[5] > self._deep_min) else 0
         view = L.TrainView(cam.viewmatrix.data_ptr(), cam.projmatrix.data_ptr(), cam.campos.data_ptr(), cam.tanfovx, cam.tanfovy,
                            gt.data_ptr(), need, need_out, self.hint_margin, self._chunk_grid(key), order, order_out, deep)
+        if phases & 3:
+            bufs = [self.params.flat_grad, self._send] + ([self.viewspace_grad] if self.densify_stats else [])
+            stamp = tuple(t._version for t in bufs)
+            if stamp != getattr(self, "_rows_stamp", None) or getattr(self.params, "_grad_rows_owner", None) is not self._rows_token:
+                self._lib.sgr_trainer_invalidate_rows(self._h)
+            self._rows_stamp = stamp
+            self.params._grad_rows_owner = self._rows_token
         with torch.cuda.device(self.dev):
             stream = C.c_void_p(torch.cuda.current_stream(self.dev).cuda_stream)
             if exchange_step is not None:
```

Measured after the change: 1081 images/s, median of 6. 1.9% higher.
